# XuyangGuo/CtrlHair

Hardware: AMD Instinct MI355X
Metric: 512x512 edited images/sec (SEAN generator forward), whole job (higher is better)
Workload: dtype f32 (every product and sum an IEEE f32 operation on the f32 matrix cores, v_mfma_f32_16x16x4_f32 / 32x32x2_f32; 3x3 convs as Winograd: ResBlock convs and the <= 64-pixel SPADE / style convs F(4x4,3x3), SPADE / style convs above F(2x2,3x3) -- f32 operands and accumulation over TRANSFORMED operands, n; 1 GPU; SEAN generator forward only, batch 16/GPU, 512x512, ngf=64 (BASELINE.json configs[1] per GPU); global_batch=16, parallelism=batch-sharded x1, labels=blocky, spade_interior_reduction=True

## Files before the change

ctrlhair_amd/csrc/ch_api.cpp:

```cpp
#include "../../include/ctrlhair_hip.h"

#include <hip/hip_runtime.h>

#include <algorithm>
#include <cmath>
#include <cstdint>
#include <cstring>
#include <new>
#include <string>

#include "aux_models.h"
#include "sean_model.h"
#include "kernels.h"
#include "png_inflate_core.h"

struct ch_handle {
    int device = 0;
    std::string err;
    chk::TensorStore tensors[4];
    chk::SeanModel sean;
    bool sean_ready = false;
    chk::ShapeModel shape;
    chk::ColorModel color;
    chk::BiSeNetModel bisenet;
// ... 643 lines not shown
int ch_sean_set_tap(ch_handle* h, const char* name, float* dev_ptr) {
    if (!h || !name) return CH_ERR_ARG;
    if (dev_ptr) h->sean.taps[name] = dev_ptr;
    else h->sean.taps.erase(name);
    return CH_OK;
}

int ch_sean_scale_report(ch_handle* h, float* host_out, int n) {
    if (!h || !host_out || n < 0) return CH_ERR_ARG;
    if (!h->sean_ready || !h->sean.amax_slots) return fail(h, CH_ERR_STATE, "ch_sean_scale_report: SEAN weights not finalized");
    DeviceGuard guard(h->device);
    unsigned raw[64];
    if (hipDeviceSynchronize() != hipSuccess ||
        hipMemcpy(raw, h->sean.amax_slots, sizeof raw, hipMemcpyDeviceToHost) != hipSuccess)
        return fail(h, CH_ERR_HIP, "ch_sean_scale_report: device read failed");
    for (int i = 0; i < n; ++i) {
        float v = 0.f;
        if (i < 64) std::memcpy(&v, &raw[i], 4);
        host_out[i] = v;
    }
    return CH_OK;
}

int ch_sean_debug_read(ch_handle* h, void* host_out, size_t bytes) {
    if (!h || !host_out) return CH_ERR_ARG;
    if (!h->sean_ready || !h->sean.splitk_ws) return fail(h, CH_ERR_STATE, "ch_sean_debug_read: SEAN weights not finalized");
    DeviceGuard guard(h->device);
    if ((long long)bytes > h->sean.splitk_cap * 4) return fail(h, CH_ERR_ARG, "ch_sean_debug_read: too many bytes");
    if (hipDeviceSynchronize() != hipSuccess || hipMemcpy(host_out, h->sean.splitk_ws, bytes, hipMemcpyDeviceToHost) != hipSuccess)
        return fail(h, CH_ERR_HIP, "ch_sean_debug_read: device read failed");
    return CH_OK;
}

}

namespace {
enum OptFreeze { NEVER, BY_SEAN, BY_SHAPE, BY_BISENET };
enum OptMap { BOOL, CLAMP, RAW };
struct OptRow {
    const char* key;
    OptFreeze frozen_by;
    OptMap map;
    int lo, hi;
    void (*set)(ch_handle*, int);
    int (*guard)(ch_handle*, int);
};
constexpr int MAXI = 0x7fffffff;
#define OPT_FIELD(field) [](ch_handle* h, int v) { h->field = v; }, nullptr
#define SEAN_FIELD(field) OPT_FIELD(sean.opt.field)

int guard_sparse(ch_handle* h, int value) {
    if (h->sean_ready && value != 0 && !h->sean.gtab)
        return fail(h, CH_ERR_STATE, "ch_set_option(sean.sparse = 1): the handle was finalised with sean.sparse = 0 (no buffers); set it before ch_finalize");
    return CH_OK;
}
int guard_dbg(ch_handle* h, int value) {
#ifndef CH_ABLATE
    if (value & CH_ABLATE_DBG_MASK)
        return fail(h, CH_ERR_ARG, "ch_set_option(sean.dbg): timing-ablation / superseded-kernel bits need a library built with -DCH_ABLATE "
                                   "(make -C ctrlhair_amd/csrc ABLATE=1)");
#endif
    return CH_OK;
}

const OptRow OPTION_TABLE[] = {
    {"sean.f16x3", BY_SEAN, RAW, 0, 0, [](ch_handle* h, int v) { h->sean.opt.use_sh16 = v != 0; h->sean.opt.terms = v == 2 ? 1 : (v == 3 ? 2 : 3); }, nullptr},
    {"shape.f16x3", BY_SHAPE, BOOL, 0, 0, OPT_FIELD(shape.use_sh16)},
    {"shape.overlap", BY_SHAPE, BOOL, 0, 0, OPT_FIELD(shape.overlap)},
    {"shape.enc_lut", BY_SHAPE, BOOL, 0, 0, OPT_FIELD(shape.enc_l0_lut)},
    {"bisenet.f16x3", BY_BISENET, BOOL, 0, 0, OPT_FIELD(bisenet.use_sh16)},
    {"aux.wino", NEVER, BOOL, 0, 0, [](ch_handle* h, int v) { h->shape.wino = h->bisenet.wino = v; }, nullptr},
    {"sean.ahead", BY_SEAN, RAW, 0, 0, [](ch_handle* h, int v) { h->sean.opt.ahead_pixels = (long long)v * 512 * 512; }, nullptr},
    {"sean.wino", BY_SEAN, CLAMP, 0, 2, SEAN_FIELD(wino)},
    {"sean.lut_grouped", BY_SEAN, BOOL, 0, 0, SEAN_FIELD(lut_grouped)},
    {"sean.prologue", BY_SEAN, BOOL, 0, 0, SEAN_FIELD(prologue)},
    {"sean.overlap", BY_SEAN, CLAMP, 0, MAXI, SEAN_FIELD(overlap)},
    {"sean.wino4_force", NEVER, BOOL, 0, 0, SEAN_FIELD(wino4_force)},
    {"sean.patch", BY_SEAN, BOOL, 0, 0, SEAN_FIELD(patch)},
    {"sean.convt_gemm", BY_SEAN, BOOL, 0, 0, SEAN_FIELD(convt_gemm)},
    {"sean.edge", BY_SEAN, BOOL, 0, 0, SEAN_FIELD(edge)},
    {"sean.frame", BY_SEAN, BOOL, 0, 0, SEAN_FIELD(frame)},
    {"sean.int_groups", NEVER, CLAMP, 0, MAXI, SEAN_FIELD(int_groups)},
    {"sean.int_onepass", NEVER, BOOL, 0, 0, SEAN_FIELD(int_onepass)},
    {"sean.batch_invariant", NEVER, BOOL, 0, 0, SEAN_FIELD(batch_inv)},
    {"sean.wino4v", BY_SEAN, BOOL, 0, 0, SEAN_FIELD(wino4v)},
    {"sean.wino4_split", BY_SEAN, CLAMP, -1, 1, SEAN_FIELD(wino4_split)},
    {"sean.wino4_ace", BY_SEAN, CLAMP, 0, MAXI, SEAN_FIELD(wino4_ace_max_r)},
    {"sean.hidden_wq", NEVER, BOOL, 0, 0, SEAN_FIELD(hidden_wq)},
    {"sean.wino_gather", BY_SEAN, BOOL, 0, 0, SEAN_FIELD(wino_gather)},
    {"sean.wino_th", BY_SEAN, RAW, 0, 0, SEAN_FIELD(wino_th)},
    {"sean.sparse", NEVER, BOOL, 0, 0, [](ch_handle* h, int v) { h->sean.opt.sparse = v; }, guard_sparse},
    {"sean.sh16_compact", BY_SEAN, CLAMP, 0, 2, SEAN_FIELD(sh16_compact)},
    {"sean.sparse_th", BY_SEAN, RAW, 0, 0, SEAN_FIELD(sparse_th)},
    {"sean.sparse_min", BY_SEAN, RAW, 0, 0, SEAN_FIELD(sparse_min_r)},
    {"sean.dbg_sel", NEVER, RAW, 0, 0, SEAN_FIELD(dbg_sel)},
    {"sean.dbg", NEVER, RAW, 0, 0, [](ch_handle* h, int v) { h->sean.opt.dbg = v; }, guard_dbg},
};
#undef SEAN_FIELD
#undef OPT_FIELD
}

extern "C" {

int ch_set_option(ch_handle* h, const char* key, int value) {
    if (!h || !key) return CH_ERR_ARG;
    for (const OptRow& r : OPTION_TABLE) {
        if (std::strcmp(key, r.key) != 0) continue;
        const bool frozen = r.frozen_by == BY_SEAN ? h->sean_ready : r.frozen_by == BY_SHAPE ? h->shape.ready : r.frozen_by == BY_BISENET && h->bisenet.ready;
        if (frozen) return fail(h, CH_ERR_STATE, std::string("ch_set_option(") + key + ") must precede ch_finalize");
        if (int rc = r.guard ? r.guard(h, value) : CH_OK) return rc;
        r.set(h, r.map == BOOL ? value != 0 : (r.map == CLAMP ? std::max(r.lo, std::min(r.hi, value)) : value));
        return CH_OK;
    }
    return fail(h, CH_ERR_ARG, std::string("unknown option '") + key + "'");
}

int ch_mfma_peak(ch_handle* h, int kind, int ms_target, double* tflops) {
    if (!h || !tflops || kind < 0 || kind > 1 || ms_target < 1 || ms_target > 2000) return fail(h, CH_ERR_ARG, "ch_mfma_peak: bad argument");
    DeviceGuard guard(h->device);
    hipError_t e = chk::mfma_peak(kind, ms_target, tflops, nullptr);
    return e == hipSuccess ? CH_OK : fail(h, CH_ERR_HIP, std::string("ch_mfma_peak: ") + hipGetErrorString(e));
}

int ch_profile_enable(ch_handle* h, int on) {
    if (!h) return CH_ERR_ARG;
    h->sean.prof_on = on != 0;
    return CH_OK;
}

int ch_profile_read(ch_handle* h, int kind, int* launches, double* total_ms, double* flops, double* bytes) {
    return ch_profile_read_ex(h, kind, launches, total_ms, flops, nullptr, bytes);
}

int ch_profile_read_ex(ch_handle* h, int kind, int* launches, double* total_ms, double* flops, double* flops_executed,
                       double* bytes) {
    if (!h) return CH_ERR_ARG;
    DeviceGuard guard(h->device);
    int n = 0;
    double ms = 0, fl = 0, fx = 0, by = 0;
    for (auto& r : h->sean.prof) {
        if (hipEventSynchronize(r.e1) != hipSuccess) return fail(h, CH_ERR_HIP, "hipEventSynchronize failed");
        if (kind < 0 || r.kind == kind) {
            float t = 0.f;
            if (hipEventElapsedTime(&t, r.e0, r.e1) != hipSuccess) return fail(h, CH_ERR_HIP, "hipEventElapsedTime failed");
            ms += t;
            fl += r.flops;
            if (r.sp_stat) {
                int st[4] = {0, 0, 0, 0};
                if (hipMemcpy(st, r.sp_stat, sizeof st, hipMemcpyDeviceToHost) != hipSuccess)
                    return fail(h, CH_ERR_HIP, "ch_profile_read: work-list statistics read failed");
                fx += (double)st[3] * r.sp_flops_unit;
                by += r.sp_bytes_fixed + r.sp_bytes_px * (r.kind == 3 ? r.sp_npix - (double)st[1] : (double)st[1]);
            } else {
                fx += r.flops_exec >= 0.0 ? r.flops_exec : r.flops;
                by += r.bytes;
            }
            ++n;
        }
    }
    if (flops_executed) *flops_executed = fx;
    if (kind < 0) {
        for (auto& r : h->sean.prof) {
            h->sean.ev_pool.push_back(r.e0);
            h->sean.ev_pool.push_back(r.e1);
        }
        h->sean.prof.clear();
// ... 11 lines not shown
```

ctrlhair_amd/csrc/conv_inst_wino.hip:

```cpp
#include "conv_pw.h"
#include <algorithm>
#include "conv_wino.h"

namespace chk {

static int wino_num_cus() {
    static int cus[64] = {};
    int dev = 0;
    if (hipGetDevice(&dev) != hipSuccess || dev < 0 || dev >= 64) return 256;
    if (!cus[dev]) {
        int v = 0;
        if (hipDeviceGetAttribute(&v, hipDeviceAttributeMultiprocessorCount, dev) != hipSuccess || v <= 0) v = 256;
        cus[dev] = v;
    }
    return cus[dev];
}

template <class K>
static hipError_t wino_attr(K kern, int bytes, bool (&done)[64]) {
    int dev = 0;
    if (hipGetDevice(&dev) != hipSuccess || dev < 0 || dev >= 64) return hipErrorInvalidDevice;
    if (!done[dev]) {
        hipError_t e = hipFuncSetAttribute(reinterpret_cast<const void*>(kern), hipFuncAttributeMaxDynamicSharedMemorySize, bytes);
        if (e != hipSuccess) return e;
// ... 10 lines not shown
        for (int k = 1; k < ks; ++k) {
            const float4 t = reinterpret_cast<const float4*>(partial + k * slab)[i];
            a.x += t.x; a.y += t.y; a.z += t.z; a.w += t.w;
        }
        const long long e = 4 * i;
        const int x = (int)(e % W), y = (int)((e / W) % H);
        const long long bc = e / ((long long)W * H);
        const float bv = bias ? bias[bc % C] : 0.f;
        a.x += bv; a.y += bv; a.z += bv; a.w += bv;
        if (res) {
            if (res_up) {
                const float* rp = res + bc * (long long)(H >> 1) * (W >> 1) + (long long)(y >> 1) * (W >> 1) + (x >> 1);
                a.x += rp[0]; a.y += rp[0]; a.z += rp[1]; a.w += rp[1];
            } else {
                const float4 r = reinterpret_cast<const float4*>(res)[i];
                a.x += r.x; a.y += r.y; a.z += r.z; a.w += r.w;
            }
        }
        if (act != ACT_NONE) { a.x = apply_act(a.x, act); a.y = apply_act(a.y, act); a.z = apply_act(a.z, act); a.w = apply_act(a.w, act); }
        reinterpret_cast<float4*>(out)[i] = a;
    }
}

hipError_t conv_wino_plain(WinoParams p, hipStream_t s) {
    if ((!wino_supported(p.H, p.W, p.Cin) && !(wino_supported_pair16(p.B, p.H, p.W, p.Cin) && !p.reflect && !p.res_up)) || !p.zero) return hipErrorInvalidValue;
    if (p.d2s && (p.Cout % 4 || p.res || p.reflect || p.in_up || !wino_supported(p.H, p.W, p.Cin))) return hipErrorInvalidValue;
    if (p.in_up && (p.reflect || !wino_supported(p.H, p.W, p.Cin))) return hipErrorInvalidValue;
    wino_fill_launch(p);
    p.ksplit = 1;
    if (p.partial && !p.d2s && p.W % 4 == 0) {
        const int cus = wino_num_cus();
        int ks = 1;
        while (ks < 8 && 2 * ks * p.ntasks <= cus && p.nks % (2 * ks) == 0 && p.nks / (2 * ks) >= 16 &&
               (long long)2 * ks * p.B * p.Cout * p.H * p.W <= p.partial_cap)
            ks *= 2;
        if (ks > 1) {
            p.ksplit = ks;
            p.ntasks *= ks;
        }
    }
    if (p.nks / p.ksplit < wino::NST) p.claim = nullptr;
    const int grid = p.ntasks < wino_num_cus() ? p.ntasks : wino_num_cus();
    static bool d0[64] = {}, d1[64] = {}, d2[64] = {};
    if (p.d2s) {
        hipError_t e = wino_attr(wino_plain_kernel<1>, wino::LDS_BYTES, d1);
        if (e != hipSuccess) return e;
        hipLaunchKernelGGL(wino_plain_kernel<1>, dim3(grid), dim3(512), wino::LDS_BYTES, s, p);
        return hipGetLastError();
    }
    if (p.in_up) {
        hipError_t e = wino_attr(wino_plain_kernel<2>, wino::LDS_BYTES, d2);
        if (e != hipSuccess) return e;
        hipLaunchKernelGGL(wino_plain_kernel<2>, dim3(grid), dim3(512), wino::LDS_BYTES, s, p);
    } else {
        hipError_t e = wino_attr(wino_plain_kernel<0>, wino::LDS_BYTES, d0);
        if (e != hipSuccess) return e;
        hipLaunchKernelGGL(wino_plain_kernel<0>, dim3(grid), dim3(512), wino::LDS_BYTES, s, p);
    }
    if (p.ksplit > 1) {
        const long long n4 = (long long)p.B * p.Cout * p.H * p.W / 4;
        const int blocks = (int)std::min<long long>((n4 + 255) / 256, 4096);
        hipLaunchKernelGGL(wino_splitk_reduce_kernel, dim3(blocks), dim3(256), 0, s, p.partial, p.out, p.bias, p.res, p.res_up, p.act, p.ksplit, p.B, p.Cout, p.H,
                           p.W);
    }
    return hipGetLastError();
}


template <int RT>
static hipError_t launch_pw(PwParams p, hipStream_t s) {
    using Cfg = PwCfg<RT>;
    static bool d0[64] = {};
    hipError_t e = wino_attr(pw_conv_kernel<RT>, Cfg::LDS_BYTES, d0);
    if (e != hipSuccess) return e;
    const int nrt = (p.Cout + 31) / 32;
    p.nrg = (nrt + RT - 1) / RT;
    p.npt = p.HW / Cfg::PXB;
    p.ntasks = p.B * p.npt * p.nrg;
    p.nst = p.Cin / 16;
    const int grid = p.ntasks < wino_num_cus() ? p.ntasks : wino_num_cus();
    hipLaunchKernelGGL(pw_conv_kernel<RT>, dim3(grid), dim3(512), Cfg::LDS_BYTES, s, p);
    return hipGetLastError();
}
hipError_t conv_pw(PwParams p, hipStream_t s) {
    if (!pw_supported(p.Cin, p.Cout, p.HW)) return hipErrorInvalidValue;
    p.groups = nullptr;
    p.ngroups = 0;
    return (p.Cout + 31) / 32 >= 4 ? launch_pw<4>(p, s) : launch_pw<2>(p, s);
}
hipError_t conv_pw_grouped(PwParams p, int ntasks, hipStream_t s) {
    using Cfg = PwCfg<4>;
    if (p.Cin % 16 || p.Cout < 1 || !p.groups || p.ngroups < 1 || ntasks < 1) return hipErrorInvalidValue;
    static bool d0[64] = {};
    hipError_t e = wino_attr(pw_conv_kernel<4>, Cfg::LDS_BYTES, d0);
    if (e != hipSuccess) return e;
    p.in = p.wpk = nullptr;
    p.out = nullptr;
    p.B = 1;
    p.HW = 0;
    p.nrg = ((p.Cout + 31) / 32 + 3) / 4;
    p.npt = 0;
    p.ntasks = ntasks;
    p.nst = p.Cin / 16;
    const int grid = ntasks < wino_num_cus() ? ntasks : wino_num_cus();
    hipLaunchKernelGGL(pw_conv_kernel<4>, dim3(grid), dim3(512), Cfg::LDS_BYTES, s, p);
    return hipGetLastError();
}

template <int TH>
static hipError_t launch_wino_ace(const WinoAceParams& p, hipStream_t s) {
    static bool d0[64] = {};
    hipError_t e = wino_attr(wino_ace_kernel<TH>, WaCfg<TH>::LDS_BYTES, d0);
    if (e != hipSuccess) return e;
    hipLaunchKernelGGL(wino_ace_kernel<TH>, dim3(wino_num_cus()), dim3(512), WaCfg<TH>::LDS_BYTES, s, p);
    return hipGetLastError();
}
hipError_t conv_wino_ace(WinoAceParams p, hipStream_t s) {
    if (p.gq) {
        if (!p.gq_n || p.gq_cap <= 0 || p.B > 32 || !p.work || !p.total || (p.C & 3) || (p.W & 1) || (p.H & 1)) return hipErrorInvalidValue;
        p.nrt = (p.C + 15) / 16;
        if (p.nrt > 2 * 65535) return hipErrorInvalidValue;
        p.K = 128 + (p.wsty ? 20 : 0);
        static bool d0[64] = {};
        hipError_t e = wino_attr(wino_ace_gather_kernel<0>, winog::LDS_BYTES, d0);
        if (e != hipSuccess) return e;
        hipLaunchKernelGGL(wino_ace_gather_kernel<0>, dim3(wino_num_cus()), dim3(512), winog::LDS_BYTES, s, p);
        return hipGetLastError();
    }
    if ((p.TH != 16 && p.TH != 32) || p.H % p.TH || p.W % wino::TW || !p.zero || !p.qlist || !p.qcnt || !p.work || !p.total || (p.C & 3))
        return hipErrorInvalidValue;
    p.nrt = (p.C + 15) / 16;
    p.ntx = p.W / wino::TW;
    p.nty = p.H / p.TH;
    p.K = 128 + (p.wsty ? 20 : 0);
    return p.TH == 32 ? launch_wino_ace<32>(p, s) : launch_wino_ace<16>(p, s);
}

__device__ __forceinline__ void wino_gather_scan_block(const int* __restrict__ qcnt, int* __restrict__ qoff, int* __restrict__ gq_n, int tps, int b) {
    __shared__ int wsum[16];
    __shared__ int carry;
    const int tid = threadIdx.x, lane = tid & 63, wave = tid >> 6;
    if (tid == 0) carry = 0;
    __syncthreads();
    for (int t0 = 0; t0 < tps; t0 += 1024) {
        const int t = t0 + tid;
        const int c = t < tps ? qcnt[b * tps + t] : 0;
        int v = c;
#pragma unroll
        for (int off = 1; off < 64; off <<= 1) {
            const int u = __shfl_up(v, off, 64);
            if (lane >= off) v += u;
        }
        if (lane == 63) wsum[wave] = v;
        __syncthreads();
        int base = carry;
        for (int w = 0; w < wave; ++w) base += wsum[w];
        if (t < tps) qoff[b * tps + t] = base + v - c;
        __syncthreads();
        if (tid == 1023) carry = base + v;
        __syncthreads();
    }
    if (tid == 0) gq_n[b] = carry;
}
__global__ __launch_bounds__(1024) void wino_gather_scan_kernel(const int* __restrict__ qcnt, int* __restrict__ qoff, int* __restrict__ gq_n, int tps) {
    wino_gather_scan_block(qcnt, qoff, gq_n, tps, (int)blockIdx.x);
}
__device__ __forceinline__ void wino_gather_fill_block(const uint8_t* __restrict__ qlist, const int* __restrict__ qcnt, const int* __restrict__ qoff,
                                                       unsigned* __restrict__ gq, int gq_cap, int ntx, int nty, int tile) {
    const int i = threadIdx.x;
    if (i >= qcnt[tile]) return;
    const int b = tile / (ntx * nty), tr = tile % (ntx * nty);
    const int q = qlist[(long long)tile * 128 + i];
    const unsigned y = (unsigned)((tr / ntx) * 16 + 2 * (q >> 4)), x = (unsigned)((tr % ntx) * 32 + 2 * (q & 15));
    gq[(long long)b * gq_cap + qoff[tile] + i] = y << 16 | x;
}
__global__ __launch_bounds__(128) void wino_gather_fill_kernel(const uint8_t* __restrict__ qlist, const int* __restrict__ qcnt, const int* __restrict__ qoff,
                                                               unsigned* __restrict__ gq, int gq_cap, int ntx, int nty) {
    wino_gather_fill_block(qlist, qcnt, qoff, gq, gq_cap, ntx, nty, (int)blockIdx.x);
}
hipError_t wino_gather_lists(const uint8_t* qlist, const int* qcnt, int* qoff, unsigned* gq, int* gq_n, int gq_cap, int B, int H, int W, hipStream_t s) {
    if (H % 16 || W % 32 || B > 32 || H > 65535 || W > 65535) return hipErrorInvalidValue;
    const int ntx = W / 32, nty = H / 16;
    hipLaunchKernelGGL(wino_gather_scan_kernel, dim3(B), dim3(1024), 0, s, qcnt, qoff, gq_n, ntx * nty);
    hipLaunchKernelGGL(wino_gather_fill_kernel, dim3(B * ntx * nty), dim3(128), 0, s, qlist, qcnt, qoff, gq, gq_cap, ntx, nty);
    return hipGetLastError();
}
__device__ __forceinline__ void wino_gather_worklist_block(const int* __restrict__ gq_n, const int* __restrict__ pcnt, int B, int tps, int nrt,
                                                           unsigned* __restrict__ work, int* __restrict__ total) {
// ... 265 lines not shown
```

ctrlhair_amd/csrc/conv_inst_wino4.hip:

```cpp
#include "conv_wino4v.h"
#include "conv_wino4_split.h"

namespace chk {

hipError_t conv_wino4_plain(Wino4Params p, hipStream_t s) {
    if (!wino4_supported(p.H, p.W, p.Cin) || !p.in || !p.wpk || !p.out || (p.reflect && (p.res_up || p.H < 2 || p.W < 2))) return hipErrorInvalidValue;
    wino4_fill_launch(p);
    static bool done[64] = {};
    static int cus[64] = {};
    int dev = 0;
    if (hipGetDevice(&dev) != hipSuccess || dev < 0 || dev >= 64) return hipErrorInvalidDevice;
    if (!done[dev]) {
        hipError_t e = hipFuncSetAttribute(reinterpret_cast<const void*>(wino4_plain_kernel<0>), hipFuncAttributeMaxDynamicSharedMemorySize, wino4::LDS_BYTES);
        if (e != hipSuccess) return e;
        e = hipFuncSetAttribute(reinterpret_cast<const void*>(wino4_plain_kernel<1>), hipFuncAttributeMaxDynamicSharedMemorySize, wino4::LDS_BYTES);
        if (e != hipSuccess) return e;
        e = hipFuncSetAttribute(reinterpret_cast<const void*>(wino4_plain_split_kernel<0>), hipFuncAttributeMaxDynamicSharedMemorySize, wino4::LDS_BYTES);
        if (e != hipSuccess) return e;
        e = hipFuncSetAttribute(reinterpret_cast<const void*>(wino4_plain_split_kernel<1>), hipFuncAttributeMaxDynamicSharedMemorySize, wino4::LDS_BYTES);
        if (e != hipSuccess) return e;
        int v = 0;
        if (hipDeviceGetAttribute(&v, hipDeviceAttributeMultiprocessorCount, dev) != hipSuccess || v <= 0) v = 256;
        cus[dev] = v;
        done[dev] = true;
    }
    const int grid = p.ntasks < cus[dev] ? p.ntasks : cus[dev];
    if (p.wpk_split && (p.split > 0 || (p.split < 0 && wino4_split_pays(p)))) {
        if (p.nks & 1) return hipErrorInvalidValue;
        if (p.reflect) hipLaunchKernelGGL(wino4_plain_split_kernel<1>, dim3(grid), dim3(512), wino4::LDS_BYTES, s, p);
        else hipLaunchKernelGGL(wino4_plain_split_kernel<0>, dim3(grid), dim3(512), wino4::LDS_BYTES, s, p);
        return hipGetLastError();
    }
    if (p.reflect) hipLaunchKernelGGL(wino4_plain_kernel<1>, dim3(grid), dim3(512), wino4::LDS_BYTES, s, p);
    else hipLaunchKernelGGL(wino4_plain_kernel<0>, dim3(grid), dim3(512), wino4::LDS_BYTES, s, p);
    return hipGetLastError();
}

hipError_t conv_wino4_ace(Wino4AceParams p, hipStream_t s) {
    if (!wino4_ace_supported(p.H, p.W, p.C) || !p.actv || !p.wpk || !p.out || !p.x || !p.noise) return hipErrorInvalidValue;
    p.nrt = (p.C + 15) / 16;
    p.ntx = p.W / wino4::TS;
    p.nty = p.H / wino4::TS;
    p.ntiles = p.B * p.ntx * p.nty;
    p.ntasks = p.ntiles * p.nrt;
    p.nks = p.wsty ? 38 : 32;
    p.rb = p.nrt >= 4 ? 4 : p.nrt;
    p.tbk = 32 / p.rb;
    static bool done[64] = {};
    static int cus[64] = {};
    int dev = 0;
    if (hipGetDevice(&dev) != hipSuccess || dev < 0 || dev >= 64) return hipErrorInvalidDevice;
    if (!done[dev]) {
        hipError_t e = hipFuncSetAttribute(reinterpret_cast<const void*>(wino4_ace_kernel<0>), hipFuncAttributeMaxDynamicSharedMemorySize, wino4::LDS_BYTES);
        if (e != hipSuccess) return e;
        int v = 0;
        if (hipDeviceGetAttribute(&v, hipDeviceAttributeMultiprocessorCount, dev) != hipSuccess || v <= 0) v = 256;
        cus[dev] = v;
        done[dev] = true;
    }
    const int grid = p.ntasks < cus[dev] ? p.ntasks : cus[dev];
    hipLaunchKernelGGL(wino4_ace_kernel<0>, dim3(grid), dim3(512), wino4::LDS_BYTES, s, p);
    return hipGetLastError();
}

__global__ __launch_bounds__(256) void wino4_style_pack_kernel(const float* __restrict__ lut, float* __restrict__ wsty, int B, int C, int nrt) {
    const long long n = (long long)B * nrt * 6 * 1152;
    const long long i = blockIdx.x * 256LL + threadIdx.x;
    if (i >= n) return;
    const int lane = (int)(i & 63), idx = (int)((i >> 6) % 18), s = (int)((i / 1152) % 6);
    const int rt = (int)((i / (1152 * 6)) % nrt), b = (int)(i / (1152LL * 6 * nrt));
    const int j = 4 * s + (lane >> 4);
    float4 o = make_float4(0.f, 0.f, 0.f, 0.f);
    const int m = (4 * idx) / 36;
    int ch, beta;
    wino4_ace_row(rt * 32 + m * 16 + (lane & 15), ch, beta);
    if (ch < C && j < 19 && s < 5) {
        const float* P = lut + ((long long)(b * 19 + j) * 9) * 2 * C + beta * C + ch;
        float g[3][3];
#pragma unroll
        for (int t = 0; t < 9; ++t) g[t / 3][t % 3] = P[(long long)t * 2 * C];
        const float Gm[6][3] = {{0.25f, 0.f, 0.f}, {-1.f / 6, -1.f / 6, -1.f / 6}, {-1.f / 6, 1.f / 6, -1.f / 6},
                                {1.f / 24, 1.f / 12, 1.f / 6}, {1.f / 24, -1.f / 12, 1.f / 6}, {0.f, 0.f, 1.f}};
        float u[4];
#pragma unroll
        for (int e = 0; e < 4; ++e) {
            const int xi = 4 * idx + e - 36 * m, ii = xi / 6, jj = xi % 6;
            float r[3];
#pragma unroll
            for (int q = 0; q < 3; ++q) r[q] = Gm[ii][0] * g[0][q] + Gm[ii][1] * g[1][q] + Gm[ii][2] * g[2][q];
            u[e] = r[0] * Gm[jj][0] + r[1] * Gm[jj][1] + r[2] * Gm[jj][2];
        }
        o = make_float4(u[0], u[1], u[2], u[3]);
    }
    reinterpret_cast<float4*>(wsty)[i] = o;
}
hipError_t wino4_style_pack(const float* lut, float* wsty, int B, int C, hipStream_t s) {
    const int nrt = (C + 15) / 16;
    const long long n = (long long)B * nrt * 6 * 1152;
    hipLaunchKernelGGL(wino4_style_pack_kernel, dim3((unsigned)((n + 255) / 256)), dim3(256), 0, s, lut, wsty, B, C, nrt);
    return hipGetLastError();
}


static hipError_t wino4v_device(int& cus) {
    static bool done[64] = {};
    static int ncu[64] = {};
    int dev = 0;
    if (hipGetDevice(&dev) != hipSuccess || dev < 0 || dev >= 64) return hipErrorInvalidDevice;
    if (!done[dev]) {
        hipError_t e = hipFuncSetAttribute(reinterpret_cast<const void*>(wino4v_kernel<0>), hipFuncAttributeMaxDynamicSharedMemorySize, wino4v::LDS_BYTES);
        if (e != hipSuccess) return e;
        e = hipFuncSetAttribute(reinterpret_cast<const void*>(wino4v_kernel<1>), hipFuncAttributeMaxDynamicSharedMemorySize, wino4v::LDS_BYTES);
        if (e != hipSuccess) return e;
        int v = 0;
        if (hipDeviceGetAttribute(&v, hipDeviceAttributeMultiprocessorCount, dev) != hipSuccess || v <= 0) v = 256;
        ncu[dev] = v;
        done[dev] = true;
    }
    cus = ncu[dev];
    return hipSuccess;
}
hipError_t wino4v_pack(const Wino4vPackParams& p, hipStream_t s) {
    if (!p.in || !p.v || p.H % 32 || p.W % 32 || p.H < 32 || p.W < 32 || p.nks <= 0 || p.pitch % 4 || p.xoff % 4 || (p.reflect && p.padded)) return hipErrorInvalidValue;
    const long long blocks = (long long)p.B * (p.H / 32) * (p.W / 32) * p.nks;
    if (blocks <= 0 || blocks > 0x7fffffffLL) return hipErrorInvalidValue;
    hipLaunchKernelGGL(wino4v_pack_kernel<0>, dim3((unsigned)blocks), dim3(256), 0, s, p);
    return hipGetLastError();
}
hipError_t conv_wino4v_plain(Wino4Params p, hipStream_t s) {
    if (!wino4_supported(p.H, p.W, p.Cin) || !p.v || !p.wpk || !p.out) return hipErrorInvalidValue;
    wino4_fill_launch(p);
    if (p.nks & 1) return hipErrorInvalidValue;
#ifndef W4V_RB
#define W4V_RB 8
#endif
    p.rb = p.nrt >= W4V_RB ? W4V_RB : p.nrt;
    p.tbk = 32 / p.rb;
    int cus = 0;
    hipError_t e = wino4v_device(cus);
    if (e != hipSuccess) return e;
    const int grid = p.ntasks < cus ? p.ntasks : cus;
    hipLaunchKernelGGL(wino4v_kernel<0>, dim3(grid), dim3(512), wino4v::LDS_BYTES, s, p);
    return hipGetLastError();
}
hipError_t conv_wino4v_ace(Wino4AceParams p, hipStream_t s) {
    if (!wino4_ace_supported(p.H, p.W, p.C) || !p.v || !p.wpk || !p.out || !p.x || !p.noise) return hipErrorInvalidValue;
    p.nrt = (p.C + 15) / 16;
    p.ntx = p.W / wino4::TS;
    p.nty = p.H / wino4::TS;
    p.ntiles = p.B * p.ntx * p.nty;
    p.ntasks = p.ntiles * p.nrt;
    p.nks = p.wsty ? 38 : 32;
    p.rb = p.nrt >= 4 ? 4 : p.nrt;
    p.tbk = 32 / p.rb;
    int cus = 0;
    hipError_t e = wino4v_device(cus);
    if (e != hipSuccess) return e;
    const int grid = p.ntasks < cus ? p.ntasks : cus;
    hipLaunchKernelGGL(wino4v_kernel<1>, dim3(grid), dim3(512), wino4v::LDS_BYTES, s, p);
    return hipGetLastError();
}

}
```

ctrlhair_amd/csrc/conv_pw.h:

```cpp
#pragma once
#include "conv_wino.h"

namespace chk {

struct PwGroup {
    const float* in;
    const float* wpk;
    float* out;
    int HW, start;
};
struct PwParams {
    const float* in;
    const float* wpk;
    float* out;
    int B, Cin, Cout, HW;
    const PwGroup* groups;
    int ngroups;
    long long in_bs;
    int nrg, npt, ntasks, nst;
};

template <class F>
std::vector<float> pack_pw_A(int rows, int Cin, F get) {
    const int nrt = (rows + 31) / 32, nst = Cin / 16;
    std::vector<float> dst((size_t)nrt * nst * 512, 0.f);
    for (int rt = 0; rt < nrt; ++rt)
        for (int st = 0; st < nst; ++st)
            for (int lane = 0; lane < 64; ++lane)
                for (int s = 0; s < 8; ++s) {
                    const int row = rt * 32 + (lane & 31), ci = 16 * st + 2 * s + (lane >> 5);
                    if (row < rows) dst[((size_t)rt * nst + st) * 512 + lane * 8 + s] = get(row, ci);
                }
    return dst;
}

template <int RT>
struct PwCfg {
    static constexpr int PG = 8 / RT, PXB = 64 * PG;
    static constexpr int PDW = 16 * PXB, ADW = RT * 512;
    static constexpr int SDW = PDW + ADW, NST = 6;
    static constexpr int NPD = PDW / (4 * 512);
    static constexpr int NLD = NPD + 1;
    static constexpr int LDS_BYTES = NST * SDW * 4 + 512 * 16;
};

template <int RT>
__global__ __launch_bounds__(512, 1) void pw_conv_kernel(const PwParams p) {
    using Cfg = PwCfg<RT>;
    constexpr int PG = Cfg::PG, PXB = Cfg::PXB, PDW = Cfg::PDW, SDW = Cfg::SDW, NST = Cfg::NST, NPD = Cfg::NPD, NLD = Cfg::NLD;
    extern __shared__ __attribute__((aligned(16))) float smem[];
    const int tid = threadIdx.x, lane = tid & 63;
    const int wave = __builtin_amdgcn_readfirstlane(tid >> 6);
    const int G = gridDim.x;
    const int lb = xcd_remap(blockIdx.x, G);
    if (lb >= p.ntasks) return;
    const int mytasks = (p.ntasks - lb + G - 1) / G;
    const int nst = p.nst;
    constexpr unsigned SB = SDW * 4, RING = NST * SB;
    auto group_of = [&](int L) {
        int g = 0;
        while (g + 1 < p.ngroups && L >= p.groups[g + 1].start * p.nrg) ++g;
        return g;
    };
    const unsigned lds0 = (unsigned)(size_t)(wino_lds_void*)smem;

    unsigned vp[NPD];
    const bool a_wave = wave < RT * 2;
    int it = lb, is = 0;
    wino_u32x4 d_in, d_a;
    unsigned so_in = 0, so_a = 0;
    int HW = p.HW;
    auto issue_task = [&]() {
        int rg, pt, ib;
        const float *tin, *twpk;
        if (p.groups) {
            const int g = group_of(it), local = it - p.groups[g].start * p.nrg;
            rg = local % p.nrg;
            pt = local / p.nrg;
            ib = 0;
            HW = p.groups[g].HW;
            tin = p.groups[g].in;
            twpk = p.groups[g].wpk;
        } else {
            rg = it % p.nrg;
            pt = (it / p.nrg) % p.npt;
            ib = it / (p.nrg * p.npt);
            tin = p.in;
            twpk = p.wpk;
        }
#pragma unroll
        for (int i = 0; i < NPD; ++i) {
            const int u = i * 512 + tid, ch = u / (PXB / 4), q = u - ch * (PXB / 4);
            vp[i] = (unsigned)(ch * HW + pt * PXB + 4 * q) * 4u;
        }
        d_in = wino_rsrc(tin + (long long)ib * (p.in_bs ? p.in_bs : (long long)p.Cin * HW), (unsigned)p.Cin * HW * 4u);
        const int nrt = (p.Cout + 31) / 32, have = nrt - rg * RT < RT ? nrt - rg * RT : RT;
        d_a = wino_rsrc(twpk + (long long)rg * RT * nst * 512, (unsigned)have * nst * 2048u);
        so_in = 0;
        so_a = 0;
    };
    issue_task();
    const unsigned va_rt = a_wave ? (unsigned)((tid >> 7) * nst * 2048 + (tid & 127) * 16) : 0x80000000u;
    unsigned islot = lds0;
    auto issue = [&]() {
        const unsigned wb = islot + (unsigned)wave * 1024u;
#pragma unroll
        for (int i = 0; i < NPD; ++i) wino_dma16(vp[i], d_in, so_in, wb + (unsigned)i * 8192u);
        const unsigned wa = a_wave ? islot + PDW * 4u + (unsigned)wave * 1024u : lds0 + RING + (unsigned)wave * 1024u;
        wino_dma16(va_rt, d_a, so_a, wa);
        islot = islot + SB == lds0 + RING ? lds0 : islot + SB;
        so_in += 64u * (unsigned)HW;
        so_a += 2048u;
        if (++is == nst) {
            if (it + G < p.ntasks) {
                it += G;
                is = 0;
                issue_task();
            } else {
                is = nst - 1;
                so_in -= 64u * (unsigned)HW;
                so_a -= 2048u;
            }
        }
    };

    f32x16 acc[2];
#pragma unroll
    for (int n = 0; n < 2; ++n)
#pragma unroll
        for (int r = 0; r < 16; ++r) acc[n][r] = 0.f;
    const int rtl = wave / PG, pg = wave % PG;
    const int boff = (lane >> 5) * PXB + pg * 64 + (lane & 31);
    const int aoff = PDW + rtl * 512 + lane * 8;

#pragma unroll
    for (int j = 0; j < NST - 1; ++j) issue();
    asm volatile("s_waitcnt vmcnt(%0)" ::"n"(NLD * (NST - 3)) : "memory");
    __syncthreads();
    unsigned rslot = lds0;
    bool after_epi = false;
    auto frag = [&](unsigned slot) { return reinterpret_cast<const float*>(smem) + (slot - lds0) / 4; };
    float4 a_lo = *reinterpret_cast<const float4*>(frag(lds0) + aoff), a_hi = *reinterpret_cast<const float4*>(frag(lds0) + aoff + 4);
    float b0 = frag(lds0)[boff], b1 = frag(lds0)[boff + 32];
    for (int k = 0, ct = lb; k < mytasks; ++k, ct += G) {
        for (int cs = 0; cs < nst; ++cs) {
            if (after_epi) asm volatile("s_waitcnt vmcnt(0)" ::: "memory");
            else asm volatile("s_waitcnt vmcnt(%0)" ::"n"(NLD * (NST - 3)) : "memory");
            __syncthreads();
            after_epi = false;
            issue();
            const unsigned nslot = rslot + SB == lds0 + RING ? lds0 : rslot + SB;
            const float* sp = frag(rslot);
            const float* spn = frag(nslot);
            const float av[8] = {a_lo.x, a_lo.y, a_lo.z, a_lo.w, a_hi.x, a_hi.y, a_hi.z, a_hi.w};
#pragma unroll
            for (int s = 0; s < 8; ++s) {
                const float c0 = b0, c1 = b1;
                if (s < 7) {
                    b0 = sp[boff + (2 * s + 2) * PXB];
                    b1 = sp[boff + (2 * s + 2) * PXB + 32];
                } else {
                    b0 = spn[boff];
                    b1 = spn[boff + 32];
                    a_lo = *reinterpret_cast<const float4*>(spn + aoff);
                    a_hi = *reinterpret_cast<const float4*>(spn + aoff + 4);
                }
                acc[0] = __builtin_amdgcn_mfma_f32_32x32x2f32(av[s], c0, acc[0], 0, 0, 0);
                acc[1] = __builtin_amdgcn_mfma_f32_32x32x2f32(av[s], c1, acc[1], 0, 0, 0);
            }
            rslot = nslot;
        }
        {
            int rg, pt, b, eHW;
            float* tout;
            if (p.groups) {
                const int g = group_of(ct), local = ct - p.groups[g].start * p.nrg;
                rg = local % p.nrg;
                pt = local / p.nrg;
                b = 0;
                eHW = p.groups[g].HW;
                tout = p.groups[g].out;
            } else {
                rg = ct % p.nrg;
                pt = (ct / p.nrg) % p.npt;
                b = ct / (p.nrg * p.npt);
                eHW = p.HW;
                tout = p.out;
            }
            const int row0 = (rg * RT + rtl) * 32 + 4 * (lane >> 5);
            float* ob = tout + (long long)b * p.Cout * eHW + pt * PXB + pg * 64 + (lane & 31);
#pragma unroll
            for (int n = 0; n < 2; ++n)
#pragma unroll
                for (int r = 0; r < 16; ++r) {
                    const int row = row0 + (r & 3) + 8 * (r >> 2);
                    if (row < p.Cout) ob[(long long)row * eHW + n * 32] = acc[n][r];
                    acc[n][r] = 0.f;
                }
            after_epi = true;
        }
    }
    asm volatile("s_waitcnt vmcnt(0)" ::: "memory");
}

inline bool pw_supported(int Cin, int Cout, int HW) { return Cin % 16 == 0 && HW % 256 == 0 && Cout >= 32; }
hipError_t conv_pw(PwParams p, hipStream_t s);
inline int pw_group_tasks(int Cout, int HW) { return ((((Cout + 31) / 32) + 3) / 4) * (HW / 128); }
hipError_t conv_pw_grouped(PwParams p, int ntasks, hipStream_t s);

}
```

ctrlhair_amd/csrc/conv_wino4.h:

```cpp
#pragma once
#include "conv_wino.h"

namespace chk {

namespace wino4 {
constexpr int TS = 32;
constexpr int PROWS = 34, PUN = 10;
constexpr int PPL = PROWS * PUN;
constexpr int PUNITS = 4 * PPL;
constexpr int PSLOTS = 1408;
constexpr int AUNITS = 1152;
constexpr int SUNITS = PSLOTS + AUNITS;
constexpr int NST = 4;
constexpr int LDS_BYTES = NST * SUNITS * 16;
constexpr int ADW = AUNITS * 4;
}

struct Wino4Params {
    const float* in;
    const float* wpk;
    float* out;
    int B, Cin, Cout, H, W;
    const float* bias;
    const float* res;
// ... 535 lines not shown
    issue_kstep();
    issue_kstep();
    asm volatile("s_waitcnt vmcnt(0)" ::: "memory");
    __syncthreads();
    unsigned rslot = lds0;
    auto kstep = [&](float (&vc)[36], float (&vx)[36]) {
        wait_ring();
        __syncthreads();
        const unsigned nslot = rslot + SB == lds0 + RING ? lds0 : rslot + SB;
        const f32x4* ap = a_ptr(rslot);
        const float* spn = stage(nslot);
        wino4_lds_f2* hbn = wino4_halo_base(spn + boff + 5);
        f32x4 F[2];
        F[0] = ap[0];
        float d[6];
        auto group = [&](auto gt) {
            constexpr int g = decltype(gt)::value;
            if constexpr (g + 1 < 9) F[(g + 1) & 1] = ap[(g + 1) * 64];
            if constexpr (g < 6) load_row(spn, hbn, g, d);
            __builtin_amdgcn_sched_barrier(0);
            const f32x4 c = F[g & 1];
            __builtin_amdgcn_s_setprio(1);
            acc[4 * g] = __builtin_amdgcn_mfma_f32_16x16x4f32(c.x, vc[4 * g], acc[4 * g], 0, 0, 0);
            acc[4 * g + 1] = __builtin_amdgcn_mfma_f32_16x16x4f32(c.y, vc[4 * g + 1], acc[4 * g + 1], 0, 0, 0);
            acc[4 * g + 2] = __builtin_amdgcn_mfma_f32_16x16x4f32(c.z, vc[4 * g + 2], acc[4 * g + 2], 0, 0, 0);
            acc[4 * g + 3] = __builtin_amdgcn_mfma_f32_16x16x4f32(c.w, vc[4 * g + 3], acc[4 * g + 3], 0, 0, 0);
            __builtin_amdgcn_s_setprio(0);
            if constexpr (g < 6)
                wino4_in1d(d[0], d[1], d[2], d[3], d[4], d[5], vx[6 * g], vx[6 * g + 1], vx[6 * g + 2], vx[6 * g + 3], vx[6 * g + 4], vx[6 * g + 5]);
            if constexpr (g >= 6) {
#pragma unroll
                for (int j = 2 * (g - 6); j < 2 * (g - 6) + 2; ++j)
                    wino4_in1d(vx[j], vx[6 + j], vx[12 + j], vx[18 + j], vx[24 + j], vx[30 + j], vx[j], vx[6 + j], vx[12 + j], vx[18 + j], vx[24 + j],
                               vx[30 + j]);
            }
            __builtin_amdgcn_sched_barrier(0);
            if constexpr (g >= 2 && g < 6) issue_piece(WInt<g - 2>{});
            __builtin_amdgcn_sched_barrier(0);
        };
        group(WInt<0>{}); group(WInt<1>{}); group(WInt<2>{}); group(WInt<3>{}); group(WInt<4>{}); group(WInt<5>{});
        group(WInt<6>{}); group(WInt<7>{}); group(WInt<8>{});
        issue_tail();
        rslot = nslot;
    };

    for (int k = 0, ct = lb; k < mytasks; ++k, ct += G) {
        {
            float v[36], w[36];
            first_v(rslot, v);
            for (int cs = 0; cs < nk; cs += 2) {
                kstep(v, w);
                kstep(w, v);
            }
        }
        int crt, tile;
        task_of(ct, crt, tile);
        wino4_ace_epilogue(p, acc, crt, tile, mh, kk, tyl, tx);
#pragma unroll
        for (int x2 = 0; x2 < 36; ++x2) acc[x2] = (f32x4){0.f, 0.f, 0.f, 0.f};
        asm volatile("s_waitcnt vmcnt(0)" ::: "memory");
    }
}

inline bool wino4_supported(int H, int W, int Cin) { return H % wino4::TS == 0 && W % wino4::TS == 0 && Cin % 8 == 0 && Cin >= 16; }
inline bool wino4_pays(long long ntasks4, int cus) {
    if (cus <= 0) cus = 256;
    const long long r4 = (ntasks4 + cus - 1) / cus, r2 = (2 * ntasks4 + cus - 1) / cus;
    return r4 * 36 * 68 < r2 * 32 * 58;
}
inline void wino4_fill_launch(Wino4Params& p) {
    p.nrt = (p.Cout + 31) / 32;
    p.ntx = p.W / wino4::TS;
    p.nty = p.H / wino4::TS;
    p.ntiles = p.B * p.ntx * p.nty;
    p.ntasks = p.ntiles * p.nrt;
    p.nks = p.Cin / 4;
    p.rb = p.nrt >= 4 ? 4 : p.nrt;
    p.tbk = 32 / p.rb;
}
inline bool wino4_split_pays(const Wino4Params& p) { return p.Cin >= 128; }
hipError_t conv_wino4_plain(Wino4Params p, hipStream_t s);
inline bool wino4_ace_supported(int H, int W, int C) { return H % wino4::TS == 0 && W % wino4::TS == 0 && C % 2 == 0; }
hipError_t conv_wino4_ace(Wino4AceParams p, hipStream_t s);
hipError_t wino4_style_pack(const float* lut, float* wsty, int B, int C, hipStream_t s);

}
```

ctrlhair_amd/csrc/kernels.h:

```cpp
#pragma once
#include <hip/hip_runtime.h>
#include <stdint.h>

#include <map>
#include <utility>
#include <vector>

namespace chk {
hipError_t label_downsample(const uint8_t* in, uint8_t* out, int B, int S, int r, hipStream_t s);
hipError_t onehot_conv3x3(const uint8_t* lab, const float* table, const float* bias, float* out, int B, int H, int W,
                          int K, int relu, hipStream_t s, int c4 = 0, const uint8_t* need = nullptr, int kout = 0);
hipError_t label_onehot_planes(const uint8_t* lab, float* out, int B, int H, int W, int kout, int k0, hipStream_t s);
bool spade_hidden_wq_supported(int H, int W);
hipError_t ace_finish_f32(const float* gb, int rowsP, const float* x, int x_up, const float* bias_g, const float* bias_b, const float* bn_a,
                          const float* bn_d, const float* nv, const float* noise, long long noise_bstride, const uint8_t* lab, const float* lut,
                          float* out, int B, int C, int H, int W, int act, hipStream_t s);
hipError_t spade_hidden_wq(const uint8_t* lab, const uint8_t* u5, const float* table, const float* bias, float* out, int B, int H, int W,
                           int kout, int onehot, hipStream_t s, int pitch = 0, int xoff = 0, const int* skip_if_patch = nullptr);
struct HiddenGroup {
    static constexpr int MAX = 24;
    struct Entry {
        const uint8_t* lab;
        const uint8_t* u5;
        const float* table;
        const float* bias;
        float* out;
        int H, W, kout, onehot, pitch, xoff;
        int tcs, start, nblk;
    };
    Entry e[MAX];
    int n, B;
};
hipError_t spade_hidden_wq_grouped(HiddenGroup& g, hipStream_t s);
hipError_t spade_hidden_patch(const uint8_t* lab, const unsigned* gq, const int* gq_n, int gq_cap, const int* chunk_base, const int* mode,
                              const float* table, const float* bias, float* patch, int B, int H, int W, int kout, hipStream_t s);
hipError_t spade_hidden_level(const uint8_t* lab, const uint8_t* u5, const unsigned* gq, const int* gq_n, int gq_cap, const int* chunk_base, const int* mode,
                              const float* table, const float* bias, float* out, float* patch, int B, int H, int W, int kout, int onehot, int pitch,
                              int xoff, hipStream_t s);
hipError_t wino_chunk_base(const int* gq_n, int B, int cap_chunks, int* chunk_base, int* mode, hipStream_t s);
hipError_t onehot_conv3x3_sh16(const uint8_t* lab, const float* table, const float* bias, void* out, int B, int H, int W,
                               int K, int relu, float scale, hipStream_t s, int bf16 = 0, const uint8_t* need = nullptr,
                               const int* tile_cnt = nullptr,
                               int need_impl = 0);
hipError_t sh16_decode(const void* in, float* out, int B, int C, long long HW, float scale, const unsigned* amax,
                       hipStream_t s, int bf16 = 0, int single = 0);
hipError_t fc_mu(const float* codes, const float* Wt, const float* bias, float* mu_img, int B, int Npad, hipStream_t s,
                 float* mu_rows = nullptr, int sh16 = 0, int bs = 19, float scale = 1.f, unsigned* amax = nullptr,
                 int pass = 0, int bf16 = 0);
hipError_t fc_mu_batched(const float* codes, const float* const* Wts, const float* const* biases, float* mu_base,
                         long long mu_stride, int n_aces, int B, int Npad, int bs, float scale, unsigned* amax_slots, int pass,
                         int bf16, hipStream_t s, int sh16 = 1);
hipError_t conv_img_tanh(const float* x, const float* w, const float* bias, float* out, int B, int Cin, int H, int W,
                         hipStream_t s, int c4 = 0, const float* w4 = nullptr);
hipError_t c4_decode(const float* in, float* out, int B, int C, long long HW, hipStream_t s);
hipError_t gen_noise(float* out, long long n, uint64_t seed, hipStream_t s);
hipError_t mfma_peak(int kind, int ms_target, double* tflops, hipStream_t s);
float instnorm_sh16_scale(int HW);
hipError_t instnorm_act(float* x, int planes, int HW, float eps, int act, hipStream_t s, void* sh16 = nullptr, int C = 0,
                        float* scratch = nullptr);
hipError_t convt_shift4(const float* x, float* xs, int B, int C, int H, int W, hipStream_t s);
hipError_t instnorm_act_d2s(const float* t, const float* bias, float* out, int B, int C, int H, int W, float eps, int act, hipStream_t s);
hipError_t instnorm_c4_to_sh16(const float* x_c4, int B, int C, int HW, float eps, int act, void* sh16, hipStream_t s,
                               float* scratch = nullptr);
hipError_t layernorm_act(float* x, const float* gamma, const float* beta, float* part, int B, int C, int HW, float eps,
                         int act, hipStream_t s);
hipError_t layernorm_act_conv(const float* x, int in_c4, void* out, int out_sh16, float out_scale, const float* gamma,
                              const float* beta, float* part, int B, int C, int HW, float eps, int act, hipStream_t s);
hipError_t region_mean(const float* codes, const uint8_t* lab, float* out, int B, int F, int h, int w, int S,
                       hipStream_t s, int c4 = 0);
hipError_t maxpool3x3s2(const float* in, float* out, long long planes, int H, int W, hipStream_t s);
hipError_t global_avg_pool(const float* in, float* out, int planes, int HW, hipStream_t s);
hipError_t chan_affine(const float* in, const float* sc, float sc_add, const float* sh, const float* other, float* out,
                       long long planes, int HW, hipStream_t s);
hipError_t stem7x7(const float* in, const float* w, const float* bias, float* out, int B, int H, int W, hipStream_t s);
hipError_t conv3x3_c3_reflect(const float* in, const float* w, const float* bias, float* out, int B, int Cout, int H, int W,
                              hipStream_t s);
hipError_t bilinear_argmax(const float* lg, uint8_t* out, float* logits_out, const uint8_t* remap, int B, int h, int w,
                           int H, int W, hipStream_t s, int c4 = 0);
hipError_t maxpool3x3s2_c4(const float* in_nchw, float* out_c4, unsigned* amax, int B, int C, int H, int W, hipStream_t s);
hipError_t global_avg_pool_c4(const float* in, float* out, int B, int C, int HW, hipStream_t s);
hipError_t chan_affine_c4(const float* in, const float* sc, float sc_add, const float* sh, const float* other, float* out,
                          unsigned* amax, int B, int C, int HW, hipStream_t s);
hipError_t shape_softmax(const float* hair, const float* face, uint8_t* lab, float* probs, int B, int HW, hipStream_t s,
                         int c4 = 0);
hipError_t c4_rows_to_nchw(const float* in, float* out, int B, int C, int Cpad, int HW, hipStream_t s);
hipError_t shape_enc_l0(const uint8_t* lab, const float* tab, const float* pc_hair, const float* pc_face, float* out_hair, float* out_face,
                        int B, int S, hipStream_t s);
hipError_t shape_inputs(const uint8_t* lab, const float* pos, float* hair_in, float* face_in, int B, int HW,
                        hipStream_t s);
hipError_t shape_inputs_sh16(const uint8_t* lab, const float* pos, void* hair_in, void* face_in, int B, int HW, float scale,
                             hipStream_t s);
hipError_t linear(const float* x, const float* W, const float* bias, const float* scale, const float* shift, float* out,
                  int B, int K, int O, int ldx, int ldo, int act, hipStream_t s);
hipError_t lut_gemv_mfma(const float* x, const float* W, float* out, int N, int rows, hipStream_t s);
hipError_t subspace_add(float* h, const float* z, int zld, const float* U, const float* L, const float* mu, int B, int D,
                        int Z, hipStream_t s);
size_t poisson_workspace_bytes(int H, int W);
hipError_t poisson_blend_batch(const uint8_t* src_hwc, const uint8_t* tgt_hwc, const uint8_t* mask, uint8_t* out_hwc, int B, int H, int W,
                               int with_gamma, int max_iters, double rel_tol, void* ws, int* iters_out, hipStream_t s);
hipError_t blend_mask_batch(const uint8_t* target_parsing, const uint8_t* face_parsing, uint8_t* out, int B, int H, int W, hipStream_t s);

constexpr int HAIR_ERODE_MAX_R = 15;
constexpr int HAIR_COLOR_NSTAT = 22;
struct HairErodeRows {
    int r;
    int hw[2 * HAIR_ERODE_MAX_R + 1];
};
hipError_t resize_linear_u8(const uint8_t* src, uint8_t* dst, int B, int Hs, int Ws, int C, int Hd, int Wd, hipStream_t s);
hipError_t hair_erode(const uint8_t* labels, int B, int Hl, int Wl, int label, const HairErodeRows& rows, uint8_t* mask, int H, int W,
                      hipStream_t s);
hipError_t hair_color_stats(const uint8_t* img, const uint8_t* mask, int B, int H, int W, int64_t* sums, hipStream_t s);

constexpr int SWEEP_NSTAT = 16;
hipError_t sheet_compose(const void* src, int kind, int n, int Hs, int Ws, const int* cells, const uint8_t* lut, uint8_t* canvas, int rows,
                         int cols, int H, int W, int margin, hipStream_t s);
hipError_t sweep_stats(const void* img, int kind, const uint8_t* labels, const int* ref, int N, int H, int W, int h, int w, int64_t* stats,
                       hipStream_t s);

constexpr int WARP_MAX_V = 2048;
constexpr int WARP_MAX_F = 4096;
constexpr int WARP_DESC_PAIRS = 16;
struct WarpDesc {
    int n, pair0;
    int d[WARP_DESC_PAIRS][6];
};
size_t mask_warp_workspace_bytes(int B);
hipError_t mask_warp_batch(const uint8_t* hair_labels, const uint8_t* face_labels, const float* V, const int* F, const int* bidx,
                           const float* bc, const int* desc_host, const float* U_in, uint8_t* labels_out, float* uv_out, float* U_out,
                           void* ws, int B, int outer_iters, int max_cg, float rel_tol, hipStream_t s);
hipError_t mask_warp_batch_dev(const uint8_t* hair_labels, const uint8_t* face_labels, const float* V, const int* F, const int* bidx,
                               const float* bc, const int* desc_dev, const float* U_in, uint8_t* labels_out, float* uv_out, float* U_out,
                               void* ws, int B, int outer_iters, int max_cg, float rel_tol, hipStream_t s);

constexpr int DELAUNAY_DESC_SETS = 64;
// ... 72 lines not shown
```

ctrlhair_amd/csrc/sean_kernels.hip:

```cpp
#include "kernels.h"
#include "sh16.h"

namespace chk {

constexpr int AF_CG = 8;
__global__ __launch_bounds__(256) void ace_finish_f32_kernel(const float* __restrict__ gb, int rowsP, const float* __restrict__ x, int x_up,
                                                             const float* __restrict__ bias_g, const float* __restrict__ bias_b,
                                                             const float* __restrict__ bn_a, const float* __restrict__ bn_d,
                                                             const float* __restrict__ nv, const float* __restrict__ noise, long long noise_bstride,
                                                             const uint8_t* __restrict__ lab, const float* __restrict__ lut, float* __restrict__ out,
                                                             int B, int C, int H, int W, int act) {
    const int HW = H * W, ppb = (HW + 255) / 256;
    const int b = blockIdx.x / ppb, pix = (blockIdx.x - b * ppb) * 256 + threadIdx.x;
    if (pix >= HW) return;
    const int y = pix / W, xx = pix - y * W;
    const int c0 = blockIdx.y * AF_CG;
    const int xW = W >> x_up, xHW = xW * (H >> x_up);
    const float nz = noise[(long long)b * noise_bstride + (long long)xx * H + y];
    const float* xp = x + ((long long)b * C + c0) * xHW + (y >> x_up) * xW + (xx >> x_up);
    const float* gp = gb + (long long)b * rowsP * HW + pix;
    float* op = out + ((long long)b * C + c0) * HW + pix;
    unsigned lo[9];
    unsigned lmask = 0;
    const float* Lb = lut ? lut + (long long)b * 19 * 9 * 2 * C : nullptr;
// ... 695 lines not shown
                        const float4 r0 = rr[0], r1 = rr[1];
                        a0.x += r0.x; a0.y += r0.y; a0.z += r0.z; a0.w += r0.w;
                        a1.x += r1.x; a1.y += r1.y; a1.z += r1.z; a1.w += r1.w;
                    }
                }
                const float v8[8] = {a0.x, a0.y, a0.z, a0.w, a1.x, a1.y, a1.z, a1.w};
                h8 vh, vl;
#pragma unroll
                for (int e2 = 0; e2 < 8; ++e2) {
                    float v = v8[e2];
                    if (relu) v = v > 0.f ? v : 0.f;
                    if (k0 + gq * 8 + e2 >= K) v = 0.f;
                    _Float16 h, l;
                    sh16_split_any(v, scale, bf16, h, l);
                    vh[e2] = h;
                    vl[e2] = l;
                }
                const long long unit = (((long long)b * G + g) * 2) * HW + pix;
                typedef unsigned u32x4 __attribute__((ext_vector_type(4)));
                __builtin_nontemporal_store(__builtin_bit_cast(u32x4, vh), reinterpret_cast<u32x4*>(out + unit));
                __builtin_nontemporal_store(__builtin_bit_cast(u32x4, vl), reinterpret_cast<u32x4*>(out + unit + HW));
            }
        }
        __syncthreads();
        if (threadIdx.x == 0) pcount = 0;
        __syncthreads();
    }
}

hipError_t onehot_conv3x3_sh16(const uint8_t* lab, const float* table, const float* bias, void* out, int B, int H, int W,
                               int K, int relu, float scale, hipStream_t s, int bf16, const uint8_t* need, const int* tile_cnt,
                               int need_impl) {
    if (need && !tile_cnt && (need_impl == 0 ? W >= 512 : need_impl == 2)) {
        const int ntile = B * ((W + 31) / 32) * ((H + 31) / 32), ky = (K + OH_KC - 1) / OH_KC;
        int gx = 1280 / ky;
        if (gx > ntile) gx = ntile;
        hipLaunchKernelGGL(onehot_conv3x3_sh16_need_kernel, dim3((unsigned)gx, (unsigned)ky), dim3(256), 0, s, lab, table, bias,
                           static_cast<uint4*>(out), B, H, W, K, relu, scale, bf16, need);
        return hipGetLastError();
    }
    const long long npix = (long long)B * H * W;
    dim3 grid((unsigned)((npix + 255) / 256), (unsigned)((K + OH_KC - 1) / OH_KC));
    hipLaunchKernelGGL(onehot_conv3x3_sh16_kernel, grid, dim3(256), 0, s, lab, table, bias, static_cast<uint4*>(out), B, H,
                       W, K, relu, scale, bf16, need, tile_cnt);
    return hipGetLastError();
}

__global__ void sh16_decode_kernel(const _Float16* __restrict__ in, float* __restrict__ out, int B, int C, long long HW,
                                   float inv_scale, const unsigned* __restrict__ amax, int bf16, int single) {
    if (amax) inv_scale /= sh16_dyn_extra(*amax);
    const long long n = (long long)B * C * HW;
    const int G = (C + 7) / 8;
    for (long long i = blockIdx.x * (long long)blockDim.x + threadIdx.x; i < n; i += (long long)gridDim.x * blockDim.x) {
        const long long p = i % HW;
        const int c = (int)((i / HW) % C), b = (int)(i / (HW * C));
        const long long unit = (((long long)b * G + c / 8) * 2) * HW + p;
        if (bf16) out[i] = (float)__builtin_bit_cast(__bf16, in[unit * 8 + (c & 7)]) * inv_scale;
        else if (single) out[i] = (float)in[unit * 8 + (c & 7)] * inv_scale;
        else out[i] = ((float)in[unit * 8 + (c & 7)] + (float)in[(unit + HW) * 8 + (c & 7)]) * inv_scale;
    }
}
hipError_t sh16_decode(const void* in, float* out, int B, int C, long long HW, float scale, const unsigned* amax,
                       hipStream_t s, int bf16, int single) {
    hipLaunchKernelGGL(sh16_decode_kernel, dim3(4096), dim3(256), 0, s, static_cast<const _Float16*>(in), out, B, C, HW,
                       1.f / scale, amax, bf16, single);
    return hipGetLastError();
}

__global__ void c4_decode_kernel(const float* __restrict__ in, float* __restrict__ out, int B, int C, long long HW) {
    const long long n = (long long)B * C * HW;
    for (long long i = blockIdx.x * (long long)blockDim.x + threadIdx.x; i < n; i += (long long)gridDim.x * blockDim.x) {
        const long long p = i % HW;
        const int c = (int)((i / HW) % C), b = (int)(i / (HW * C));
        out[i] = in[(((long long)b * (C >> 2) + (c >> 2)) * HW + p) * 4 + (c & 3)];
    }
}
hipError_t c4_decode(const float* in, float* out, int B, int C, long long HW, hipStream_t s) {
    hipLaunchKernelGGL(c4_decode_kernel, dim3(4096), dim3(256), 0, s, in, out, B, C, HW);
    return hipGetLastError();
}

constexpr int FCMU_BT = 8;

__device__ __forceinline__ void fc_mu_body(const float* __restrict__ codes, const float* __restrict__ Wt,
                                           const float* __restrict__ bias, float* __restrict__ mu_img, int B, int Npad,
                                           float* __restrict__ mu_rows, int sh16, int bs, float scale,
                                           unsigned* __restrict__ amax, int pass, int bf16, int bx, int j) {
    sh16_mode_on();
    if (sh16 == 1 && amax && pass == 1) {
        const float e = sh16_dyn_extra(*amax);
        if (e == 1.f) return;
        scale *= e;
    }
    float vmax = 0.f;
    const int wave = threadIdx.x >> 6, lane = threadIdx.x & 63;
    const int o0 = (bx * 4 + wave) * 4;
    const float* Wj = Wt + (long long)j * 512 * 512;
    float4 w[4][2];
#pragma unroll
    for (int i = 0; i < 4; ++i) {
        const float4* wr = reinterpret_cast<const float4*>(Wj + (long long)(o0 + i) * 512 + lane * 8);
        w[i][0] = wr[0];
        w[i][1] = wr[1];
    }
    for (int bb = 0; bb < B; bb += FCMU_BT) {
        float part[4][FCMU_BT];
#pragma unroll
        for (int t = 0; t < FCMU_BT; ++t) {
            float4 c0 = make_float4(0, 0, 0, 0), c1 = c0;
            if (bb + t < B) {
                const float4* cr =
                    reinterpret_cast<const float4*>(codes + ((long long)(bb + t) * 19 + j) * 512 + lane * 8);
                c0 = cr[0];
                c1 = cr[1];
            }
#pragma unroll
            for (int i = 0; i < 4; ++i)
                part[i][t] = w[i][0].x * c0.x + w[i][0].y * c0.y + w[i][0].z * c0.z + w[i][0].w * c0.w +
                             w[i][1].x * c1.x + w[i][1].y * c1.y + w[i][1].z * c1.z + w[i][1].w * c1.w;
        }
#pragma unroll
        for (int i = 0; i < 4; ++i)
#pragma unroll
            for (int t = 0; t < FCMU_BT; ++t) {
                float v = part[i][t];
#pragma unroll
                for (int off = 32; off > 0; off >>= 1) v += __shfl_xor(v, off, 64);
                part[i][t] = v;
            }
        if (lane == 0) {
#pragma unroll
            for (int i = 0; i < 4; ++i)
#pragma unroll
                for (int t = 0; t < FCMU_BT; ++t)
                    if (bb + t < B) {
                        const float v = part[i][t] + bias[j * 512 + o0 + i];
                        const float r = v > 0.f ? v : 0.f;
                        const int o = o0 + i, n = (bb + t) * bs + j;
                        if (bs > 19 && j == 0) {
                            const int nz = (bb + t) * bs + 19;
                            if (mu_rows) mu_rows[(long long)nz * 512 + o] = 0.f;
                            else if (sh16 == 1) {
                                _Float16* mh = reinterpret_cast<_Float16*>(mu_img);
                                mh[(((long long)(o >> 3) * 2 + 0) * Npad + nz) * 8 + (o & 7)] = (_Float16)0.f;
                                mh[(((long long)(o >> 3) * 2 + 1) * Npad + nz) * 8 + (o & 7)] = (_Float16)0.f;
                            }
                        }
                        if (mu_rows) mu_rows[(long long)n * 512 + o] = r;
                        else if (sh16 == 2)
                            mu_img[((long long)(n >> 5) * 32 + (o >> 4)) * 512 + ((n & 31) + 32 * (o & 1)) * 8 + ((o & 15) >> 1)] = r;
                        else if (sh16) {
                            _Float16* mh = reinterpret_cast<_Float16*>(mu_img);
                            _Float16 h, l;
                            sh16_split_any(r, scale, bf16, h, l);
                            vmax = fmaxf(vmax, r * scale);
                            mh[(((long long)(o >> 3) * 2 + 0) * Npad + n) * 8 + (o & 7)] = h;
                            mh[(((long long)(o >> 3) * 2 + 1) * Npad + n) * 8 + (o & 7)] = l;
                        } else mu_img[(long long)o * Npad + n] = r;
                    }
        }
    }
    if (sh16 == 1 && amax && pass == 0 && lane == 0) sh16_slot_max(amax, vmax);
}
__global__ __launch_bounds__(256) void fc_mu_kernel(const float* __restrict__ codes, const float* __restrict__ Wt,
                                                    const float* __restrict__ bias, float* __restrict__ mu_img, int B,
                                                    int Npad, float* __restrict__ mu_rows, int sh16, int bs, float scale,
                                                    unsigned* __restrict__ amax, int pass, int bf16) {
    fc_mu_body(codes, Wt, bias, mu_img, B, Npad, mu_rows, sh16, bs, scale, amax, pass, bf16, blockIdx.x, blockIdx.y);
}
__global__ __launch_bounds__(256) void fc_mu_batched_kernel(const float* __restrict__ codes, const float* const* __restrict__ Wts,
                                                            const float* const* __restrict__ biases, float* __restrict__ mu_base,
                                                            long long mu_stride, int B, int Npad, int bs, float scale,
                                                            unsigned* __restrict__ amax_slots, int pass, int bf16, int sh16) {
    const int a = blockIdx.z;
    const float* Wt = Wts[a];
    if (!Wt) return;
    fc_mu_body(codes, Wt, biases[a], mu_base + a * mu_stride, B, Npad, nullptr, sh16, bs, scale, sh16 == 1 ? amax_slots + 2 * a + 1 : nullptr, pass,
               bf16, blockIdx.x, blockIdx.y);
}
hipError_t fc_mu_batched(const float* codes, const float* const* Wts, const float* const* biases, float* mu_base,
                         long long mu_stride, int n_aces, int B, int Npad, int bs, float scale, unsigned* amax_slots, int pass,
                         int bf16, hipStream_t s, int sh16) {
    hipLaunchKernelGGL(fc_mu_batched_kernel, dim3(512 / 16, 19, n_aces), dim3(256), 0, s, codes, Wts, biases, mu_base, mu_stride, B,
                       Npad, bs, scale, amax_slots, pass, bf16, sh16);
    return hipGetLastError();
}

hipError_t fc_mu(const float* codes, const float* Wt, const float* bias, float* mu_img, int B, int Npad,
                 hipStream_t s, float* mu_rows, int sh16, int bs, float scale, unsigned* amax, int pass, int bf16) {
    hipLaunchKernelGGL(fc_mu_kernel, dim3(512 / 16, 19), dim3(256), 0, s, codes, Wt, bias, mu_img, B, Npad, mu_rows, sh16, bs,
                       scale, amax, pass, bf16);
    return hipGetLastError();
}

constexpr int CI_TW = 32, CI_TH = 8, CI_CK = 8;

__global__ __launch_bounds__(256) void conv_img_kernel(const float* __restrict__ x, const float* __restrict__ w,
                                                       const float* __restrict__ bias, float* __restrict__ out, int B,
                                                       int Cin, int H, int W, int c4) {
    __shared__ float patch[CI_CK][CI_TH + 2][CI_TW + 2];
    const int tx = threadIdx.x % CI_TW, ty = threadIdx.x / CI_TW;
    const int x0 = blockIdx.x * CI_TW, y0 = blockIdx.y * CI_TH, b = blockIdx.z;
    const long long HW = (long long)H * W;
    float a0 = 0.f, a1 = 0.f, a2 = 0.f;
    for (int c0 = 0; c0 < Cin; c0 += CI_CK) {
        __syncthreads();
        for (int e = threadIdx.x; e < CI_CK * (CI_TH + 2) * (CI_TW + 2); e += 256) {
            const int c = e / ((CI_TH + 2) * (CI_TW + 2)), rem = e % ((CI_TH + 2) * (CI_TW + 2));
            const int py = rem / (CI_TW + 2), px = rem % (CI_TW + 2);
            const int yy = y0 + py - 1, xx = x0 + px - 1;
            float v = 0.f;
            if (c0 + c < Cin && (unsigned)yy < (unsigned)H && (unsigned)xx < (unsigned)W) {
                const int ch = c0 + c;
                v = c4 ? x[(((long long)b * (Cin >> 2) + (ch >> 2)) * HW + (long long)yy * W + xx) * 4 + (ch & 3)]
                       : x[((long long)b * Cin + ch) * HW + (long long)yy * W + xx];
                v = v > 0.f ? v : 0.2f * v;
            }
            patch[c][py][px] = v;
        }
        __syncthreads();
        const float* w0 = w + (long long)c0 * 9;
#pragma unroll
        for (int c = 0; c < CI_CK; ++c) {
            if (c0 + c >= Cin) break;
#pragma unroll
            for (int t = 0; t < 9; ++t) {
                const float v = patch[c][ty + t / 3][tx + t % 3];
                a0 += w0[c * 9 + t] * v;
                a1 += w0[(long long)Cin * 9 + c * 9 + t] * v;
                a2 += w0[(long long)Cin * 18 + c * 9 + t] * v;
            }
        }
    }
    const int xx = x0 + tx, yy = y0 + ty;
    if (xx < W && yy < H) {
        float* o = out + (long long)b * 3 * HW + (long long)yy * W + xx;
        o[0] = tanhf(a0 + bias[0]);
        o[HW] = tanhf(a1 + bias[1]);
        o[2 * HW] = tanhf(a2 + bias[2]);
    }
}

template <bool NCHW>
__global__ __launch_bounds__(256) void conv_img_c4_kernel(const float4* __restrict__ x, const float4* __restrict__ w4,
                                                          const float* __restrict__ bias, float* __restrict__ out, int B,
                                                          int Cin, int H, int W) {
    constexpr int PW = CI_TW + 2, PH = CI_TH + 2, NP = PW * PH;
    __shared__ float4 patch[2][NP];
    const int G = Cin >> 2;
    const int tx = threadIdx.x % CI_TW, ty = threadIdx.x / CI_TW;
    const int x0 = blockIdx.x * CI_TW, y0 = blockIdx.y * CI_TH, b = blockIdx.z;
    const long long HW = (long long)H * W;
    int off[2];
#pragma unroll
    for (int i = 0; i < 2; ++i) {
        const int e = threadIdx.x + i * 256;
        const int py = e / PW, px = e % PW, yy = y0 + py - 1, xx = x0 + px - 1;
        off[i] = (e < NP && (unsigned)yy < (unsigned)H && (unsigned)xx < (unsigned)W) ? yy * W + xx : -1;
    }
    const float4* xb = x + (long long)b * G * HW;
    const float* xp = reinterpret_cast<const float*>(x) + (long long)b * Cin * HW;
    float4 r[2];
    auto fetch = [&](int g) {
#pragma unroll
        for (int i = 0; i < 2; ++i) {
            float4 v;
            if constexpr (NCHW) {
                const float* q = xp + (long long)(4 * g) * HW + (off[i] >= 0 ? off[i] : 0);
                v = make_float4(q[0], q[HW], q[2 * HW], q[3 * HW]);
            } else {
                v = xb[(long long)g * HW + (off[i] >= 0 ? off[i] : 0)];
            }
            r[i] = off[i] >= 0 ? v : make_float4(0.f, 0.f, 0.f, 0.f);
// ... 82 lines not shown
```

ctrlhair_amd/csrc/sean_model.cpp:

```cpp
#include "sean_model.h"

#include <cmath>
#include <cstring>
#include <type_traits>

#include "ace_sparse.h"
#include "conv_ace_sparse.h"
#include "conv_mfma.h"
#include "conv_sh16.h"
#include "conv_pw.h"
#include "conv_wino.h"
#include "conv_wino4v.h"
#include "kernels.h"
#include "sh16.h"

namespace chk {

size_t SeanModel::noise_floats(int S) const {
    size_t n = 0;
    for (const auto& b : blocks) {
        const size_t r = (size_t)S / b.res_div;
        n += r * r * (b.learned ? 3 : 2);
    }
    return n;
// ... 549 lines not shown
            m.ev_int.assign(n_aces, nullptr);
            for (auto& e : m.ev_x)
                if (hipEventCreateWithFlags(&e, hipEventDisableTiming) != hipSuccess) return "event creation failed";
            for (auto& e : m.ev_int)
                if (hipEventCreateWithFlags(&e, hipEventDisableTiming) != hipSuccess) return "event creation failed";
            m.claim_pool = static_cast<unsigned*>(B.dalloc((size_t)SeanModel::CLAIM_SLOTS * SeanModel::CLAIM_WORDS * sizeof(unsigned)));
        }
        m.ahead_limit = limit;
        if (limit <= 0) return "";
        m.ahead_full = m.overlap_on || (long long)mb * ms * ms <= limit;
        if (!m.overlap_on && (hipStreamCreateWithFlags(&m.side, hipStreamNonBlocking) != hipSuccess || hipEventCreateWithFlags(&m.ev_fork, hipEventDisableTiming) != hipSuccess))
            return "side stream creation failed";
        m.ev_join.assign(n_aces, nullptr);
        m.actv_ahead.assign(n_aces, nullptr);
        m.lut_ahead.assign(n_aces, nullptr);
        for (auto& e : m.ev_join)
            if (hipEventCreateWithFlags(&e, hipEventDisableTiming) != hipSuccess) return "event creation failed";
        for_each_ace(m.blocks, [&](const AceW& a) {
            const size_t r = (size_t)ms / a.res_div;
            if (m.ahead_full) m.actv_ahead[a.index] = B.falloc((size_t)mb * r * (r + 64) * (HID + 20));
            if (a.styled) m.lut_ahead[a.index] = B.falloc(npad() * 18 * a.C);
        });
        m.splitk_side = B.falloc((size_t)m.splitk_cap);
        return "";
    }

    size_t npad() const { return (((size_t)mb * (LABEL_NC + 1) + 31) / 32) * 32; }
    std::string arena() {
        const size_t MB = mb, S = ms;
        for (int k = 1; k <= 5; ++k) {
            const size_t r = S >> k;
            m.lab_r[k] = static_cast<uint8_t*>(B.dalloc(MB * r * r));
        }
        size_t nf = m.noise_floats(ms);
        m.noise_ws = static_cast<float*>(B.dalloc(MB * nf * 4));
        m.mu_img = static_cast<float*>(B.dalloc((size_t)STYLE * npad() * 4));
        if (m.mu_img) (void)hipMemset(m.mu_img, 0, (size_t)STYLE * npad() * 4);
        style_projections();
        style_lut_groups();
        size_t lutmax = 0, h0max = 0, midmax = 0, outmax = 0;
        for (const auto& b : m.blocks) {
            const size_t r = S / b.res_div, px = MB * r * r;
            if (b.styled) lutmax = std::max(lutmax, npad() * 18 * b.fin);
            h0max = std::max(h0max, px * b.fin);
            midmax = std::max(midmax, px * b.fmid);
            outmax = std::max(outmax, px * b.fout);
        }
        outmax = std::max(outmax, (size_t)MB * 16 * m.ngf * (S / 32) * (S / 32));
        if (m.has_zencoder) {
            h0max = std::max(h0max, MB * S * S * 128);
            midmax = std::max(midmax, MB * S * S * (opt.use_sh16 ? 64 : 16));
        }
        m.lut = static_cast<float*>(B.dalloc(lutmax * 4));
        m.actv = static_cast<float*>(B.dalloc(MB * S * S * HID * 4));
        m.h0 = static_cast<float*>(B.dalloc(h0max * 4));
        m.hs = static_cast<float*>(B.dalloc(h0max * 4));
        m.dx = static_cast<float*>(B.dalloc(midmax * 4));
        m.h1 = static_cast<float*>(B.dalloc(midmax * 4));
        m.xs = static_cast<float*>(B.dalloc(outmax * 4));
        m.xa = static_cast<float*>(B.dalloc(outmax * 4));
        m.xb = static_cast<float*>(B.dalloc(outmax * 4));
        return "";
    }
    void style_projections() {
        const int n_aces = m.n_aces;
        m.fcmu_batched = opt.use_sh16 ? mb * (LABEL_NC + 1) > 64 : mb * LABEL_NC > 64;
        if (!m.fcmu_batched) return;
        m.mu_stride = (long long)STYLE * npad();
        m.mu_all = static_cast<float*>(B.dalloc((size_t)n_aces * m.mu_stride * 4));
        if (m.mu_all) (void)hipMemset(m.mu_all, 0, (size_t)n_aces * m.mu_stride * 4);
        std::vector<const float*> wp(n_aces, nullptr), bp(n_aces, nullptr);
        for_each_ace(m.blocks, [&](const AceW& a) {
            if (a.styled) { wp[a.index] = a.fcmu_w; bp[a.index] = a.fcmu_b; }
        });
        m.fcmu_w_ptrs = static_cast<const float**>(B.dalloc(n_aces * sizeof(float*)));
        m.fcmu_b_ptrs = static_cast<const float**>(B.dalloc(n_aces * sizeof(float*)));
        if (m.fcmu_w_ptrs && m.fcmu_b_ptrs) {
            (void)hipMemcpy(m.fcmu_w_ptrs, wp.data(), n_aces * sizeof(float*), hipMemcpyHostToDevice);
            (void)hipMemcpy(m.fcmu_b_ptrs, bp.data(), n_aces * sizeof(float*), hipMemcpyHostToDevice);
        }
    }
    void style_lut_groups() {
        m.lut_groups = nullptr;
        m.lut_ngroups = m.lut_group_tiles = 0;
        m.lut_group_rows = 0.0;
        if (!(m.fcmu_batched && !opt.use_sh16 && opt.lut_grouped)) return;
        if (m.lut_ahead.empty()) m.lut_ahead.assign(m.n_aces, nullptr);
        std::vector<PwGroup> g;
        bool ok = true;
        for_each_ace(m.blocks, [&](const AceW& a) {
            if (a.styled && (!a.lut_wt || (18 * a.C) % 128)) ok = false;
        });
        for_each_ace(m.blocks, [&](const AceW& a) {
            if (!ok || !a.styled) return;
            if (!m.lut_ahead[a.index]) m.lut_ahead[a.index] = B.falloc(npad() * 18 * a.C);
            PwGroup e{};
            e.in = a.lut_wt;
            e.wpk = m.mu_all + (size_t)a.index * m.mu_stride;
            e.out = m.lut_ahead[a.index];
            e.HW = 18 * a.C;
            e.start = m.lut_group_tiles;
            if (!e.out) { ok = false; return; }
            m.lut_group_tiles += e.HW / 128;
            m.lut_group_rows += e.HW;
            g.push_back(e);
        });
        if (ok && !g.empty()) {
            m.lut_groups = B.dalloc(g.size() * sizeof(PwGroup));
            if (m.lut_groups) (void)hipMemcpy(m.lut_groups, g.data(), g.size() * sizeof(PwGroup), hipMemcpyHostToDevice);
            m.lut_ngroups = (int)g.size();
        }
    }

    std::string wino_levels() {
        for (int k = 0; k < 6; ++k) {
            m.wq_level[k] = SeanModel::WinoLevel();
            m.actv_lvl[k] = nullptr;
        }
        m.pad_state.clear();
        m.wsty = m.wsty4 = nullptr;
        if (!(opt.wino && !opt.use_sh16)) return "";
        size_t wsty_max = 0, wsty4_max = 0;
        int lvl_planes[6] = {0, 0, 0, 0, 0, 0};
        for_each_ace(m.blocks, [&](const AceW& a) {
            if (!a.spade_wino) return;
            const int k = level_of(a.res_div), r = ms >> k;
            if (r < 32 || r % 32) return;
            SeanModel::WinoLevel& L = m.wq_level[k];
            if (!L.qlist) wino_level_lists(L, r);
            const int nrt = (a.C + 15) / 16;
            bool have = false;
            for (const auto& w : L.works) have = have || w.nrt == nrt;
            if (!have) {
                SeanModel::WinoWork w;
                w.nrt = nrt;
                w.work = static_cast<unsigned*>(B.dalloc(((size_t)L.cap_tiles * 4 + mb) * ((nrt + 1) / 2) * sizeof(unsigned)));
                w.total = static_cast<int*>(B.dalloc(8 * sizeof(int)));
                L.works.push_back(w);
            }
            lvl_planes[k] = std::max(lvl_planes[k], a.styled ? HID + 20 : HID);
            if (a.styled) wsty_max = std::max(wsty_max, (size_t)mb * nrt * 5 * 2048);
            if (a.styled && a.spade_wino4) wsty4_max = std::max(wsty4_max, (size_t)mb * nrt * 6 * wino4::ADW);
        });
        if (wsty_max) m.wsty = B.falloc(wsty_max);
        m.patchbuf = nullptr;
        m.patch_cap_chunks = 0;
        if (opt.patch && opt.wino_gather && mb <= 32) {
            m.patch_cap_chunks = 32 * mb;
            m.patchbuf = B.falloc((size_t)m.patch_cap_chunks * (HID + 20) * 1024);
        }
        if (wsty4_max) m.wsty4 = B.falloc(wsty4_max);
        wino4v_buffer();
        for (int k = 0; k < 6; ++k)
            if (m.wq_level[k].qlist) {
                const size_t r = (size_t)ms >> k;
                m.actv_lvl[k] = B.falloc((size_t)mb * r * wino_apitch((int)r) * lvl_planes[k]);
            }
        return "";
    }
    void wino_level_lists(SeanModel::WinoLevel& L, int r) {
        const bool gather = opt.wino_gather && mb <= 32 && (r / 2) * (r / 2) <= 2048 * 64;
        L.TH = gather ? 16 : opt.wino_tile_h(r);
        L.cap_tiles = mb * (r / 32) * (r / L.TH);
        L.qlist = static_cast<uint8_t*>(B.dalloc((size_t)L.cap_tiles * 8 * L.TH));
        L.qcnt = static_cast<int*>(B.dalloc((size_t)L.cap_tiles * sizeof(int)));
        L.pcnt = static_cast<int*>(B.dalloc((size_t)L.cap_tiles * sizeof(int)));
        if (gather) {
            L.gq_cap = (r / 2) * (r / 2);
            L.gq = static_cast<unsigned*>(B.dalloc((size_t)mb * L.gq_cap * sizeof(unsigned)));
            L.gq_n = static_cast<int*>(B.dalloc(32 * sizeof(int)));
            L.qoff = static_cast<int*>(B.dalloc((size_t)L.cap_tiles * sizeof(int)));
            L.chunk_base = static_cast<int*>(B.dalloc(34 * sizeof(int)));
            L.patch_mode = static_cast<int*>(B.dalloc(sizeof(int)));
        }
    }
    void wino4v_buffer() {
        m.vbuf = nullptr;
        m.vbuf_bytes = 0;
        if (!(opt.wino >= 2 && opt.wino4v)) return;
        size_t need = 0;
        auto level_r = [&](int res_div) {
            const int r = ms >> level_of(res_div);
            return (r < 32 || r % 32 || r > 64) ? 0 : r;
        };
        for (const auto& b : m.blocks)
            for (const ConvW* c : {&b.conv_0, &b.conv_1})
                if (const int r = level_r(b.res_div))
                    if (c->wino4 && wino4v_pays(c->Cout, r)) need = std::max(need, wino4v_bytes(mb, r, r, c->Cin / 4));
        for_each_ace(m.blocks, [&](const AceW& a) {
            if (const int r = level_r(a.res_div))
                if (m.ace_route_shape(a, r) == AceRoute::F4 && wino4v_pays(2 * a.C, r)) need = std::max(need, wino4v_bytes(mb, r, r, 38));
        });
        if (m.z14_wino4 && (ms / 2) % 32 == 0 && wino4v_bytes(mb, ms / 2, ms / 2, 64) <= ((size_t)5 << 29)) need = std::max(need, wino4v_bytes(mb, ms / 2, ms / 2, 64));
        if (need) {
            m.vbuf = static_cast<float*>(B.dalloc(need));
            m.vbuf_bytes = need;
        }
    }

    std::string sparse_levels() {
        m.prof_stats_cap = 16384;
        m.prof_stats_used = 0;
        m.prof_stats = static_cast<int*>(B.dalloc((size_t)m.prof_stats_cap * 4 * sizeof(int)));
        for (int k = 0; k < 6; ++k) {
            m.sp_level[k][0] = m.sp_level[k][1] = SparseLevel();
            m.sp_work[k].clear();
        }
        m.gtab = m.gtab_side = nullptr;
        if (!opt.sparse) return "";
        int cmax = 0;
        for_each_ace(m.blocks, [&](const AceW& a) {
            const int k = level_of(a.res_div), r = ms >> k;
            if (r < opt.sparse_min_r || r < 32) return;
            const int mt = (a.C + 31) / 32;
            const int th = opt.use_sh16 ? 16 : opt.sparse_tile_h(mt, r);
            SparseLevel& L = m.sp_level[k][th == 16 ? 1 : 0];
            if (!L.u5) {
                L.TH = th;
                L.cap_tiles = mb * ((r + 31) / 32) * ((r + L.TH - 1) / L.TH);
                L.u5 = static_cast<uint8_t*>(B.dalloc((size_t)mb * r * r));
                L.e16 = (opt.edge && (opt.use_sh16 || opt.wino) && r >= 128) ? static_cast<uint16_t*>(B.dalloc((size_t)mb * r * r * sizeof(uint16_t))) : nullptr;
                L.need = static_cast<uint8_t*>(B.dalloc((size_t)mb * r * r));
                L.list = static_cast<uint16_t*>(B.dalloc((size_t)L.cap_tiles * 32 * L.TH * sizeof(uint16_t)));
                L.cnt = static_cast<int*>(B.dalloc((size_t)L.cap_tiles * sizeof(int)));
            }
            bool have = false;
            for (const auto& w : m.sp_work[k]) have = have || w.mtiles == mt;
            if (!have) {
                SparseWork w;
                w.mtiles = mt;
                w.TH = L.TH;
                w.mode = opt.use_sh16 ? (opt.sh16_compact ? (opt.sh16_compact >= 2 ? 2 : 3) : 1) : 0;
                w.cap = (long long)L.cap_tiles * (opt.use_sh16 ? mt : sparse_max_tasks(L.TH, mt));
                w.work = static_cast<unsigned*>(B.dalloc((size_t)w.cap * sizeof(unsigned)));
// ... 284 lines not shown
            } else {
                check(wino_quad_lists(o.S ? o.S->u5 : nullptr, L.qlist, L.qcnt, L.pcnt, B, r, r, L.TH, st), "wino_quad_lists");
                if (L.gq) check(wino_gather_lists(L.qlist, L.qcnt, L.qoff, L.gq, L.gq_n, L.gq_cap, B, r, r, st), "wino_gather_lists");
                if (L.gq && L.chunk_base) check(wino_chunk_base(L.gq_n, B, m.patchbuf ? m.patch_cap_chunks : 0, L.chunk_base, L.patch_mode, st), "wino_chunk_base");
            }
            ls.wq_done = true;
        }
        bool done = false;
        for (int d : ls.wwork_done) done = done || d == nrt;
        if (!done) {
            if (geo && ls.geo_slot >= 0 && geo->nw < WinoGeoGroup::MAX_W) {
                WinoGeoGroup::Work& w = geo->w[geo->nw++];
                w.level = ls.geo_slot;
                w.nrt = nrt;
                w.work = p.W->work;
                w.total = p.W->total;
            } else {
                if (geo && ls.geo_slot >= 0) geo_flush();
                if (L.gq) check(wino_gather_worklist(L.gq_n, L.pcnt, B, ntiles / B, nrt, p.W->work, p.W->total, st), "wino_gather_worklist");
                else check(wino_ace_worklist(L.qcnt, L.pcnt, ntiles, nrt, p.W->work, p.W->total, st), "wino_ace_worklist");
            }
            ls.wwork_done.push_back(nrt);
        }
        return o;
    }
    WinoGeoGroup* geo = nullptr;
    void geo_flush() {
        if (!geo) return;
        if (geo->nl) check(wino_geometry_grouped(*geo, st), "level geometry (grouped)");
        geo->nl = geo->nw = 0;
        for (LevelState& s : lvl) s.geo_slot = -1;
    }
    const uint8_t* level_u5(const AcePlan& p) const {
        if (!m.opt.sparse || p.r < m.opt.sparse_min_r) return nullptr;
        for (int ti = 1; ti >= 0; --ti)
            if (m.sp_level[p.k][ti].u5 && lvl[p.k].done[ti]) return m.sp_level[p.k][ti].u5;
        return nullptr;
    }
    std::vector<AcePlan> plans;
    void plan_aces(const uint8_t* labfull) {
        plans.assign(m.n_aces, AcePlan());
        for_each_ace(m.blocks, [&](const AceW& a) {
            AcePlan& p = plans[a.index];
            p.a = &a;
            p.k = level_of(a.res_div);
            p.r = S / a.res_div;
            p.lab = a.res_div == 1 ? labfull : m.lab_r[p.k];
            p.route = m.ace_route(a, p.r, B);
            p.abuf = (p.wino() && m.actv_lvl[p.k]) ? m.actv_lvl[p.k] : m.actv;
            p.kout = a.styled ? HID + 20 : HID;
            p.ahead.lut_ns = 18 * a.C;
            if (p.wino()) {
                p.L = &m.wq_level[p.k];
                p.W = m.wino_work(a, p.r);
                if (p.route == AceRoute::WinoQuads && p.L->gq && mode.ahead != SeanModel::ChunkMode::FULL && m.patchbuf && !mode.overlap) p.patch = p.L;
                return;
            }
            p.sw = m.sparse_work(a, p.r);
            if (p.route != AceRoute::Sparse) return;
            p.SL = &m.sp_level[p.k][p.sw->TH == 16 ? 1 : 0];
            p.compact = m.opt.use_sh16 && p.sw->mode >= 2;
            if (mode.ahead == SeanModel::ChunkMode::FULL) return;
            if (m.opt.use_sh16 ? p.compact : (m.opt.dbg & 131072) != 0) p.need = p.SL->need;
            if (m.opt.use_sh16 && !p.compact) p.tile_cnt = p.SL->cnt;
        });
    }
    void prepass() {
        for (const AcePlan& p : plans)
            if (p.route == AceRoute::WinoQuads) (void)wino_prepare(p);
    }

    AcePrep build_lut(const AcePlan& pl, const float* codes, hipStream_t s, float* lut_buf, float* splitk, bool prof) {
        const AceW& a = *pl.a;
        AcePrep q;
        q.lut_ns = 18 * a.C;
        if (!a.styled) return q;
        q.lut = lut_buf;
        const int bs = m.opt.use_sh16 ? LABEL_NC + 1 : LABEL_NC;
        const int N = B * bs, npad = ((N + 31) / 32) * 32;
        q.lut_bs = bs;
        const double fl = 2.0 * 18 * a.C * STYLE * N, by = 4.0 * (18.0 * a.C * STYLE + (double)STYLE * N + 18.0 * a.C * N);
        auto tm = [&](auto launch) { prof ? timed(2, fl, by, launch) : launch(); };
        if (a.lut_rows && N <= 64 && !m.opt.batch_inv) {
            check(fc_mu(codes, a.fcmu_w, a.fcmu_b, m.mu_img, B, npad, s, m.mu_img, 0, bs), "fc_mu");
            tm([&] { check(lut_gemv_mfma(m.mu_img, a.lut_rows, lut_buf, N, 18 * a.C, s), "lut gemv"); });
            return q;
        }
        ConvParams p{};
        p.in = m.mu_img;
        p.wpk = a.lut_wpk;
        p.out = lut_buf;
        p.B = 1;
        p.Cin = STYLE;
        p.H = npad / 32;
        p.W = 32;
        p.Mrows = 18 * a.C;
        p.pad = -1;
        if (m.opt.use_sh16) {
            unsigned* mu_slot = m.amax_slots + 2 * a.index + 1;
            if (m.fcmu_batched) {
                p.in = m.mu_all + (size_t)a.index * m.mu_stride;
            } else {
                for (int pass = 0; pass < 2; ++pass)
                    check(fc_mu(codes, a.fcmu_w, a.fcmu_b, m.mu_img, B, npad, s, nullptr, 1, bs, SH16_ACT_SCALE, mu_slot, pass, m.opt.terms == 2), "fc_mu");
            }
            p.act = ACT_NONE;
            p.terms = m.opt.terms;
            p.wscale = a.lut_wscale;
            p.in_scale_inv = 1.f / SH16_ACT_SCALE;
            p.in_amax = mu_slot;
            p.out_mul = a.out_scale;
            p.partial = splitk;
            p.partial_cap = m.splitk_cap;
            tm([&] { check(conv_sh16_plain(p, 1, s), "lut gemm"); });
            q.lut_rs = npad;
            q.lut_ns = 4;
        } else {
            if (m.fcmu_batched && (N > 64 || m.opt.batch_inv)) p.in = m.mu_all + (size_t)a.index * m.mu_stride;
            else check(fc_mu(codes, a.fcmu_w, a.fcmu_b, m.mu_img, B, npad, s), "fc_mu");
            p.npix_valid = N;
            tm([&] { check(conv_nhwc1x1(p, s), "lut gemm"); });
        }
        return q;
    }
    void zero_pads(float* buf, int r, int kout, hipStream_t s) {
        const long long geo = ((long long)r << 20) | ((long long)kout << 8) | 1;
        auto it = m.pad_state.find(buf);
        if (it != m.pad_state.end() && it->second == geo) return;
        check(hipMemsetAsync(buf, 0, (size_t)m.max_batch * kout * r * wino_apitch(r) * sizeof(float), s), "hidden activations: zero pads");
        m.pad_state[buf] = geo;
    }
    void build_hidden(const AcePlan& pl, hipStream_t s, float* actv_buf) {
        const AceW& a = *pl.a;
        const int r = pl.r, kout = pl.kout;
        const uint8_t* lab = pl.lab;
        if (!pl.wino()) m.pad_state.erase(actv_buf);
        if (m.opt.use_sh16)
            check(onehot_conv3x3_sh16(lab, a.actv_table, a.actv_bias, actv_buf, B, r, r, HID, 1, a.actv_scale, s, m.opt.terms == 2, pl.need, pl.tile_cnt,
                                      (m.opt.dbg & 33554432) ? 1 : 0), "mlp_shared");
        else if (pl.wino()) {
            zero_pads(actv_buf, r, kout, s);
            const uint8_t* u5 = (pl.route == AceRoute::WinoQuads && m.opt.hidden_wq) ? level_u5(pl) : nullptr;
            const SeanModel::WinoLevel* PL = pl.patch;
            const bool pm = PL && PL->gq && PL->patch_mode && m.patchbuf;
            if (pm && mode.prologue && PL->chunk_base) {
                check(spade_hidden_level(lab, u5, PL->gq, PL->gq_n, PL->gq_cap, PL->chunk_base, PL->patch_mode, a.actv_table,
                                         a.actv_bias, actv_buf, m.patchbuf, B, r, r, kout, a.styled ? 1 : 0, wino_apitch(r), WINO_AXOFF, s),
                      "mlp_shared (planes or pre-gathered patches)");
                return;
            }
            check(spade_hidden_wq(lab, u5, a.actv_table, a.actv_bias, actv_buf, B, r, r, kout, a.styled ? 1 : 0, s,
                                  wino_apitch(r), WINO_AXOFF, pm ? PL->patch_mode : nullptr), "mlp_shared (boundary-quad patches)");
            if (pm) check(spade_hidden_patch(lab, PL->gq, PL->gq_n, PL->gq_cap, PL->chunk_base, PL->patch_mode, a.actv_table, a.actv_bias, m.patchbuf,
                                             B, r, r, kout, s), "mlp_shared (pre-gathered patches)");
        } else
            check(onehot_conv3x3(lab, a.actv_table, a.actv_bias, actv_buf, B, r, r, HID, 1, s, 0, pl.need), "mlp_shared");
    }

    void prepare_all_ahead(const float* codes) {
        const bool full = mode.ahead == SeanModel::ChunkMode::FULL;
        check(hipEventRecord(m.ev_fork, st), "fork");
        check(hipStreamWaitEvent(m.side, m.ev_fork, 0), "fork wait");
        for (AcePlan& p : plans) {
            const AceW& a = *p.a;
            if (!full && !a.styled) continue;
            if (!(mode.grouped && a.styled)) p.ahead = build_lut(p, codes, m.side, m.lut_ahead[a.index], m.splitk_side, false);
            p.ahead.actv = m.actv_ahead[a.index];
            if (full) build_hidden(p, m.side, m.actv_ahead[a.index]);
            check(hipEventRecord(m.ev_join[a.index], m.side), "join record");
        }
    }

    void luts_grouped() {
        const int N = B * LABEL_NC;
        PwParams q{};
        q.Cin = STYLE;
        q.Cout = N;
        q.groups = static_cast<const PwGroup*>(m.lut_groups);
        q.ngroups = m.lut_ngroups;
        const int nrg = ((N + 31) / 32 + 3) / 4;
        timed(2, 2.0 * m.lut_group_rows * STYLE * N, 4.0 * (m.lut_group_rows * STYLE + m.lut_group_rows * N + (double)m.lut_ngroups * STYLE * N),
              [&] { check(conv_pw_grouped(q, m.lut_group_tiles * nrg, st), "style LUTs (grouped GEMM)"); });
        for (AcePlan& p : plans)
            if (p.a->styled) p.ahead.lut = m.lut_ahead[p.a->index];
    }

    void prologue() {
        HiddenGroup hg{};
        AceTableGroup tg{};
        StylePackGroup sg{};
        WinoGeoGroup gg{};
        hg.B = tg.B = sg.B = gg.B = B;
        geo = &gg;
        tg.lut_rs = 1;
        tg.lut_bs = LABEL_NC;
        tg.lut_mul = 1.f;
        for (AcePlan& p : plans) {
            const AceW& a = *p.a;
            const int r = p.r;
            if (p.route == AceRoute::F4) {
                float* buf = m.pro_actv[a.index];
                if (!buf || hg.n >= HiddenGroup::MAX) continue;
                zero_pads(buf, r, p.kout, st);
                HiddenGroup::Entry& e = hg.e[hg.n++];
                e.lab = p.lab;
                e.u5 = nullptr;
                e.table = a.actv_table;
                e.bias = a.actv_bias;
                e.out = buf;
                e.H = e.W = r;
                e.kout = p.kout;
                e.onehot = a.styled ? 1 : 0;
                e.pitch = wino_apitch(r);
                e.xoff = WINO_AXOFF;
                p.pre_actv = buf;
                continue;
            }
            if (p.route != AceRoute::WinoQuads) continue;
            const WinoPrep wp = wino_prepare(p);
            if (a.styled && !mode.grouped) continue;
            const float* lut = a.styled ? p.ahead.lut : nullptr;
            if (a.styled && !lut) continue;
            const bool p6 = wp.edges && a.styled;
            if (wp.S && m.pro_gtab[a.index] && (!p6 || m.pro_p6[a.index]) && tg.n < AceTableGroup::MAX) {
                AceTableGroup::Entry& e = tg.e[tg.n++];
                e.bias_g = a.bias_g;
                e.bias_b = a.bias_b;
                e.gconst = a.gconst;
                e.lut = lut;
                e.gtab = m.pro_gtab[a.index];
                e.p6 = p6 ? m.pro_p6[a.index] : nullptr;
                e.C = a.C;
                p.pre_gtab = e.gtab;
                p.pre_p6 = e.p6;
            }
            if (a.styled && m.pro_wsty[a.index] && sg.n < StylePackGroup::MAX) {
                StylePackGroup::Entry& e = sg.e[sg.n++];
                e.lut = lut;
                e.wsty = m.pro_wsty[a.index];
                e.C = a.C;
                p.pre_wsty = e.wsty;
            }
        }
        geo_flush();
        geo = nullptr;
        check(spade_hidden_wq_grouped(hg, st), "mlp_shared (grouped, F(4x4)-route ACEs)");
        check(ace_tables_grouped(tg, st), "ace tables (grouped)");
        check(wino_style_pack_grouped(sg, st), "wino_style_pack (grouped)");
    }

    void ace(const AceW& a, const float* codes, const float* noise, size_t nf, size_t noff, const float* x, int x_up, int act, float* hout) {
        const AcePlan& p = plans[a.index];
        const AceIO io{noise + noff, (long long)nf, x, x_up, act, hout};
        const WinoPrep wp = p.route == AceRoute::WinoQuads ? wino_prepare(p) : WinoPrep();
        if (p.sw) sparse_prepare(p);
        const AcePrep q = operands(p, codes);
        switch (p.route) {
            case AceRoute::F4: return ace_f4(p, q, io);
            case AceRoute::WinoQuads: return ace_wino(p, wp, q, io);
            case AceRoute::Sparse: return ace_sparse(p, q, io);
            case AceRoute::TinySplitK: return ace_tiny(p, q, io);
            case AceRoute::Dense: return ace_dense(p, q, io);
        }
    }
    AcePrep operands(const AcePlan& p, const float* codes) {
        const AceW& a = *p.a;
        AcePrep q;
        if (mode.ahead == SeanModel::ChunkMode::FULL) {
            q = p.ahead;
            check(hipStreamWaitEvent(st, m.ev_join[a.index], 0), "join wait");
        } else {
            const bool lut_made = a.styled && (mode.grouped || mode.ahead == SeanModel::ChunkMode::LUTS);
            if (!lut_made) q = build_lut(p, codes, st, m.lut, m.splitk_ws, true);
            if (!p.pre_actv) build_hidden(p, st, p.abuf);
            if (lut_made) q = p.ahead;
            q.actv = p.abuf;
            if (lut_made && !mode.grouped) check(hipStreamWaitEvent(st, m.ev_join[a.index], 0), "join wait");
        }
        if (p.pre_actv) q.actv = p.pre_actv;
        return q;
    }
    template <class P>
    void fill_mod(P& t, const AcePlan& p, const AceIO& io) {
        const AceW& a = *p.a;
        t.x = io.x;
        t.x_up = io.x_up;
        t.act = io.act;
        t.out = io.out;
        t.B = B;
        t.C = a.C;
        t.H = t.W = p.r;
        t.bn_a = a.bn_a;
        t.bn_d = a.bn_d;
        t.nv = a.nv;
        t.noise = io.noise;
        t.noise_bstride = io.nf;
        if constexpr (!std::is_same<P, AceInteriorParams>::value) {
            t.bias_g = a.bias_g;
            t.bias_b = a.bias_b;
        }
    }
    AceInteriorParams interior_params(const AcePlan& p, const AceIO& io, const SparseLevel& L) {
        AceInteriorParams ip{};
        fill_mod(ip, p, io);
        ip.u5 = L.u5;
        ip.cnt = L.cnt;
        ip.gtab = m.gtab;
        return ip;
    }
    void interior_edges(AceInteriorParams& ip, const AcePlan& p, const AcePrep& q, const SparseLevel& L) {
        ip.e16 = L.e16;
        ip.etab = p.a->edge_tab;
        ip.p6 = (p.a->styled && q.lut) ? m.p6 : nullptr;
    }
    double dense_flops(const AcePlan& p) const { return 2.0 * 2 * p.a->C * HID * 9 * ((double)B * p.r * p.r); }

    void ace_f4(const AcePlan& p, const AcePrep& q, const AceIO& io) {
        const AceW& a = *p.a;
        const int r = p.r;
        const double npix = (double)B * r * r;
        Wino4AceParams w{};
        fill_mod(w, p, io);
        w.actv = q.actv;
        w.wpk = a.spade_wino4;
        w.wsty = (a.styled && q.lut) ? m.wsty4 : nullptr;
        const int nks = w.wsty ? 38 : 32, ktot = 4 * nks;
        next_flops_exec = 2.0 * 32.0 * ((a.C + 15) / 16) * ktot * 36.0 * npix / 16.0;
        Wino4vPackParams vp;
        const bool vroute = m.wino4v_route(wino4v_pays(2 * a.C, r), q.actv, B, r, p.kout, nks, vp, true);
        timed(1, dense_flops(p), 4.0 * (npix * p.kout + npix * a.C / (io.x_up ? 4.0 : 1.0) + npix * a.C), [&] {
            if (w.wsty) check(wino4_style_pack(q.lut, m.wsty4, B, a.C, st), "wino4_style_pack");
            if (vroute) {
                check(wino4v_pack(vp, st), "hidden activation transform (winograd F(4x4,3x3))");
                w.v = m.vbuf;
                check(conv_wino4v_ace(w, st), "spade conv (winograd F(4x4,3x3), every tile, pre-transformed input)");
            } else
                check(conv_wino4_ace(w, st), "spade conv (winograd F(4x4,3x3), every tile)");
        });
    }
    void ace_wino(const AcePlan& p, const WinoPrep& wp, const AcePrep& q, const AceIO& io) {
        const AceW& a = *p.a;
        const int r = p.r, x_up = io.x_up;
        const double npix = (double)B * r * r;
        const double xpp = 4.0 * a.C / (x_up ? 4.0 : 1.0), opp = 4.0 * a.C;
        const int ktot = p.kout;
        if (wp.S) {
            AceInteriorParams ip = interior_params(p, io, *wp.S);
            ip.impl = r >= 128 ? 2 : 0;
            ip.groups = m.opt.int_groups;
            ip.onepass = m.opt.int_onepass;
            if (wp.edges) {
                if (!a.edge_tab || r < 128) check(hipErrorInvalidValue, "straight-edge marks on a level whose ACE has no table");
                interior_edges(ip, p, q, *wp.S);
            }
            ip.fill_min = (x_up && r < 128) ? 257 : ((r >= 128 && !(m.opt.dbg & 134217728)) ? 0 : 128);
            if (mode.overlap) {
                ip.fill_min = 257;
                ip.quad_only = 1;
                ip.gtab = m.gtab_side;
                check(hipEventRecord(m.ev_x[a.index], st), "x ready");
                check(hipStreamWaitEvent(m.side_int, m.ev_x[a.index], 0), "x ready wait");
                check(ace_gtable(a.bias_g, a.bias_b, a.gconst, q.lut, q.lut_rs, q.lut_ns, q.lut_bs, 1.f, m.gtab_side, B, a.C, m.side_int), "ace_gtable");
                check(ace_interior_f32(ip, m.side_int), "ace interior");
                check(hipEventRecord(m.ev_int[a.index], m.side_int), "interior done");
            } else {
                const bool pre = p.pre_gtab && (ip.p6 != nullptr) == (p.pre_p6 != nullptr);
                if (pre) {
                    ip.gtab = p.pre_gtab;
                    ip.p6 = p.pre_p6;
                }
                timed(3, 0.0, 0.0, SpStat{p.W->total + 4, 0.0, xpp + opp + 5.0, 4.0 * 19 * 2 * a.C * B, npix}, [&] {
                    if (!pre) {
                        check(ace_gtable(a.bias_g, a.bias_b, a.gconst, q.lut, q.lut_rs, q.lut_ns, q.lut_bs, 1.f, m.gtab, B, a.C, st), "ace_gtable");
                        if (ip.p6) check(ace_p6table(q.lut, q.lut_rs, q.lut_ns, q.lut_bs, 1.f, m.p6, B, a.C, st), "ace_p6table");
                    }
                    check(ace_interior_f32(ip, st), "ace interior");
                });
            }
        }
        const SeanModel::WinoLevel& L = *p.L;
        WinoAceParams w{};
        fill_mod(w, p, io);
        w.actv = q.actv;
        w.wpk = a.spade_wino;
        const float* pre_wsty = (a.styled && q.lut) ? p.pre_wsty : nullptr;
        w.wsty = (a.styled && q.lut) ? (pre_wsty ? pre_wsty : m.wsty) : nullptr;
        w.patch = p.patch ? m.patchbuf : nullptr;
        w.chunk_base = L.chunk_base;
        w.patch_mode = L.patch_mode;
        w.qlist = L.qlist;
        w.TH = L.TH;
        w.qcnt = L.qcnt;
        w.work = p.W->work;
        w.total = p.W->total;
        w.zero = m.zero_page;
        w.gq = L.gq;
        w.gq_n = L.gq_n;
        w.gq_cap = L.gq_cap;
        w.claim = w.gq ? next_claim() : nullptr;
        timed(1, dense_flops(p), 0.0, SpStat{p.W->total + 4, 2.0 * 32 * 16 * 16 * ktot, 4.0 * ktot + xpp + opp, 4.0 * 2.0 * a.C * ktot * 16, npix}, [&] {
            if (w.wsty && !pre_wsty) check(wino_style_pack(q.lut, m.wsty, B, a.C, st), "wino_style_pack");
            check(conv_wino_ace(w, st), "spade conv (winograd, boundary quads)");
        });
        if (mode.overlap && wp.S) check(hipStreamWaitEvent(st, m.ev_int[a.index], 0), "interior done wait");
    }
    ConvParams ace_conv_params(const AcePlan& pl, const AcePrep& q, const AceIO& io) {
        const AceW& a = *pl.a;
        ConvParams p{};
        fill_mod(p, pl, io);
        p.in = q.actv;
        p.wpk = a.spade_wpk;
        p.Cin = HID;
        p.Mrows = 2 * a.C;
        p.lab = pl.lab;
// ... 112 lines not shown
        p.wpk = w.wpk;
        p.out = out;
        p.B = B;
        p.Cin = w.Cin;
        p.H = r;
        p.W = r;
        p.Mrows = w.Cout;
        p.bias = w.bias;
        p.res = res;
        p.res_up = res_up;
        p.act = ACT_NONE;
        p.pad = -1;
        p.dbg = m.opt.dbg;
        p.terms = m.opt.terms;
        p.wscale = w.wscale;
        p.in_scale_inv = 1.f / prod.out_scale;
        p.partial = m.opt.batch_inv ? nullptr : m.splitk_ws;
        p.partial_cap = m.splitk_cap;
        p.mtiles_hint_small = (((w.Cout + 63) / 64) * (((long long)B * r * r + 511) / 512) < 192) ? 1 : 0;
        const double npix = (double)B * r * r, k2 = w.KS * w.KS, cin2 = w2 ? w2->Cin : 0;
        if (m.opt.wino >= 2 && !m.opt.use_sh16 && w.wino4 && w.KS == 3 && !w2 && wino4_supported(r, r, w.Cin) &&
            (!use_wino(w, r) || m.opt.wino4_force || m.opt.batch_inv || wino4_pays((long long)B * (r / 32) * (r / 32) * ((w.Cout + 31) / 32), m.num_cus))) {
            Wino4Params q{};
            q.in = in;
            q.wpk = w.wino4;
            q.out = out;
            q.B = B;
            q.Cin = w.Cin;
            q.Cout = w.Cout;
            q.H = r;
            q.W = r;
            q.bias = w.bias;
            q.res = res;
            q.res_up = res_up;
            q.wpk_split = w.wino4s;
            q.split = m.opt.wino4_split;
            next_flops_exec = 2.0 * w.Cout * w.Cin * 36.0 * npix / 16.0;
            Wino4vPackParams vp;
            const bool vroute = m.wino4v_route(wino4v_pays(w.Cout, r), in, B, r, w.Cin, w.Cin / 4, vp);
            timed(0, 2.0 * w.Cout * w.Cin * 9.0 * npix,
                  4.0 * (npix * w.Cin + npix * w.Cout * (res ? 2.0 : 1.0) + (double)w.Cout * w.Cin * 36.0), [&] {
                      if (vroute) {
                          check(wino4v_pack(vp, st), "conv input transform (winograd F(4x4,3x3))");
                          q.v = m.vbuf;
                          check(conv_wino4v_plain(q, st), "conv (winograd F(4x4,3x3), pre-transformed input)");
                      } else
                          check(conv_wino4_plain(q, st), "conv (winograd F(4x4,3x3))");
                  });
            return;
        }
        if (use_wino(w, r) && !w2 && !(r == 16 && res_up)) {
            WinoParams q{};
            q.in = in;
            q.wpk = w.wino;
            q.out = out;
            q.B = B;
            q.Cin = w.Cin;
            q.Cout = w.Cout;
            q.H = r;
            q.W = r;
            q.bias = w.bias;
            q.res = res;
            q.res_up = res_up;
            q.act = ACT_NONE;
            q.zero = m.zero_page;
            q.claim = next_claim();
            q.partial = m.opt.batch_inv ? nullptr : m.splitk_ws;
            q.partial_cap = m.splitk_cap;
            next_flops_exec = 2.0 * w.Cout * w.Cin * 16.0 * npix / 4.0;
            timed(0, 2.0 * w.Cout * w.Cin * 9.0 * npix,
                  4.0 * (npix * w.Cin + npix * w.Cout * (res ? 2.0 : 1.0) + (double)w.Cout * w.Cin * 16.0),
                  [&] { check(conv_wino_plain(q, st), "conv (winograd)"); });
            return;
        }
        if (m.opt.wino && !m.opt.use_sh16 && w.pw && w.KS == 1 && !w2 && !res && !w.bias && pw_supported(w.Cin, w.Cout, r * r)) {
            PwParams q{};
            q.in = in;
            q.wpk = w.pw;
            q.out = out;
            q.B = B;
            q.Cin = w.Cin;
            q.Cout = w.Cout;
            q.HW = r * r;
            timed(0, 2.0 * w.Cout * w.Cin * npix, 4.0 * (npix * w.Cin + npix * w.Cout + (double)w.Cout * w.Cin),
                  [&] { check(conv_pw(q, st), "conv 1x1"); });
            return;
        }
        timed(0, 2.0 * w.Cout * (w.Cin * k2 + cin2) * npix,
              4.0 * (npix * (w.Cin + cin2) + npix * w.Cout * (res ? 2.0 : 1.0) + (double)w.Cout * (w.Cin * k2 + cin2)), [&] {
                  if (m.opt.use_sh16) check(conv_sh16_plain(p, w.KS, st), "conv");
                  else check(w.KS == 3 ? conv_plain3(p, st) : conv_plain1(p, st), "conv");
              });
    }
};

}

static uint64_t chunk_seed(uint64_t seed, int bo) { return seed + 0x632BE59BD9B4E019ull * (uint64_t)(bo + 1); }

std::string SeanModel::draw_noise(uint64_t seed, float* out, int Btot, int S, hipStream_t st) {
    if (blocks.empty()) return "model not finalized";
    if (S % 32 != 0 || S < 32 || S > max_size) return "S must be a multiple of 32 and <= max_size";
    const size_t nf = noise_floats(S);
    for (int bo = 0; bo < Btot; bo += max_batch) {
        const int B = std::min(max_batch, Btot - bo);
        if (gen_noise(out + (size_t)bo * nf, (long long)B * nf, chunk_seed(seed, bo), st) != hipSuccess) return "gen_noise failed";
    }
    return "";
}

std::string SeanModel::generate(const uint8_t* labels, const float* codes, const float* noise, uint64_t seed,
                                float* out, int Btot, int S, hipStream_t st) {
    if (blocks.empty()) return "model not finalized";
    if (S % 32 != 0 || S < 32 || S > max_size) return "S must be a multiple of 32 and <= max_size";
    if (Btot < 1) return "B must be >= 1";
    const size_t nf = noise_floats(S);
    hipStream_t st_user = st;
    if (overlap_on) {
        if (hipEventRecord(ev_in, st_user) != hipSuccess || hipStreamWaitEvent(main_i, ev_in, 0) != hipSuccess) return "overlap mode: fork failed";
        st = main_i;
    }
    auto join = [&](const std::string& e) {
        if (overlap_on && (hipEventRecord(ev_out, main_i) != hipSuccess || hipStreamWaitEvent(st_user, ev_out, 0) != hipSuccess) && e.empty())
            return std::string("overlap mode: join failed");
        return e;
    };
    for (int bo = 0; bo < Btot; bo += max_batch) {
        const int B = std::min(max_batch, Btot - bo);
        const uint8_t* lab = labels + (size_t)bo * S * S;
        Runner R(*this, st, B, S, lab);
        const ChunkMode& mode = R.mode;
        if (claim_pool) R.check(hipMemsetAsync(claim_pool, 0, (size_t)CLAIM_SLOTS * CLAIM_WORDS * sizeof(unsigned), st), "claim counters");
        const float* cd = codes + (size_t)bo * LABEL_NC * STYLE;
        const float* nz;
        if (noise) {
            nz = noise + (size_t)bo * nf;
        } else {
            R.check(gen_noise(noise_ws, (long long)B * nf, chunk_seed(seed, bo), st), "gen_noise");
            nz = noise_ws;
        }
        for (int k = 1; k <= 5; ++k) R.check(label_downsample(lab, lab_r[k], B, S, S >> k, st), "label_downsample");
        if (opt.use_sh16) R.check(hipMemsetAsync(amax_slots, 0, 64 * sizeof(unsigned), st), "amax slots");
        if (mode.project_all) {
            R.check(fc_mu_batched(cd, fcmu_w_ptrs, fcmu_b_ptrs, mu_all, mu_stride, n_aces, B, ((B * LABEL_NC + 31) / 32) * 32, LABEL_NC, 1.f,
                                  nullptr, 0, 0, st, mode.grouped ? 2 : 0), "fc_mu (all ACEs)");
            if (mode.grouped) R.luts_grouped();
        } else if (fcmu_batched && opt.use_sh16) {
            const int npad_c = ((B * (LABEL_NC + 1) + 31) / 32) * 32;
            for (int pass = 0; pass < 2; ++pass)
                R.check(fc_mu_batched(cd, fcmu_w_ptrs, fcmu_b_ptrs, mu_all, mu_stride, n_aces, B, npad_c, LABEL_NC + 1, SH16_ACT_SCALE,
                                      amax_slots, pass, opt.terms == 2, st), "fc_mu (all ACEs)");
        }
        if (mode.prepass) R.prepass();
        if (mode.ahead != ChunkMode::NONE) R.prepare_all_ahead(cd);
        if (mode.prologue) R.prologue();

        const int sw = S / 32;
        float* x = xa;
        float* y = xb;
        R.check(onehot_conv3x3(lab_r[5], fc_table, fc_bias, x, B, sw, sw, 16 * ngf, 0, st, opt.use_sh16 ? 1 : 0), "fc");
        R.tap_c4("fc", x, 16 * ngf, (size_t)sw * sw);
        size_t noff = 0;
        for (const auto& b : blocks) {
            const int r = S / b.res_div;
            const size_t rr = (size_t)r * r;
            const int up = b.up_before ? 1 : 0;
            const float* xsrc = x;
            const float* shortcut;
            int sc_up;
            bool fuse_s = false;
            if (b.learned) {
                R.ace(b.ace_s, cd, nz, nf, noff, xsrc, up, ACT_NONE, hs);
                noff += rr;
                R.tap_sh16(b.name + ".hs", hs, b.fin, rr, b.ace_s);
                fuse_s = R.can_fuse_1x1(b.conv_1, r) && !taps.count(b.name + ".xs") && !R.use_wino(b.conv_1, r);
                if (!fuse_s) {
                    R.conv(b.conv_s, hs, b.ace_s, xs, r, nullptr, 0);
                    R.tap_c4(b.name + ".xs", xs, b.fout, rr);
                }
                shortcut = fuse_s ? nullptr : xs;
                sc_up = 0;
            } else {
                shortcut = xsrc;
                sc_up = up;
            }
            R.ace(b.ace_0, cd, nz, nf, noff, xsrc, up, ACT_LRELU, h0);
            noff += rr;
            R.tap_sh16(b.name + ".h0", h0, b.fin, rr, b.ace_0);
            R.conv(b.conv_0, h0, b.ace_0, dx, r, nullptr, 0);
            R.tap_c4(b.name + ".dx", dx, b.fmid, rr);
            R.ace(b.ace_1, cd, nz, nf, noff, dx, 0, ACT_LRELU, h1);
            noff += rr;
            R.tap_sh16(b.name + ".h1", h1, b.fmid, rr, b.ace_1);
            R.conv(b.conv_1, h1, b.ace_1, y, r, shortcut, sc_up, fuse_s ? &b.conv_s : nullptr, fuse_s ? hs : nullptr, fuse_s ? &b.ace_s : nullptr);
            R.tap_c4(b.name, y, b.fout, rr);
            std::swap(x, y);
        }
        R.check(conv_img_tanh(x, img_w, img_b, out + (size_t)bo * 3 * S * S, B, ngf, S, S, st, opt.use_sh16 ? 1 : 0, img_w4), "conv_img");
        if (!R.err.empty()) return join(R.err);
    }
    return join("");
}

std::string SeanModel::encode(const float* img, const uint8_t* labels, float* codes_out, int Btot, int S,
                              hipStream_t st, int phase) {
    if (blocks.empty() || !has_zencoder) return "Zencoder weights not loaded/finalized";
    if (S % 32 != 0 || S < 32 || S > max_size) return "S must be a multiple of 32 and <= max_size";
    if (phase != 0 && Btot > max_batch) return "split encode: B must not exceed max_batch";
    if (phase == 1) { enc_pending_B = Btot; enc_pending_S = S; }
    if (phase == 2 && (enc_pending_B != Btot || enc_pending_S != S)) return "split encode: no matching ch_sean_encode_features call";
    if (phase == 2) enc_pending_B = 0;
    for (int bo = 0; bo < Btot; bo += max_batch) {
        const int B = std::min(max_batch, Btot - bo);
        std::string err;
        auto ck = [&](hipError_t e, const char* what) {
            if (e != hipSuccess && err.empty()) err = std::string(what) + ": " + hipGetErrorString(e);
        };
        const float* x = img + (size_t)bo * 3 * S * S;
        ConvOpts refl;
        refl.pad_mode = PAD_REFLECT;
        ConvOpts zero;
        ConvOpts zins;
        zins.in_mode = IN_UP2_ZEROINS;
        ConvOpts last = refl;
        last.act = ACT_TANH;
        const int h2 = S / 2, h4 = S / 4;
        const bool f16path = opt.use_sh16 && h4 * h4 >= 4096;
        bool in4_done = false;
        if (phase != 2) {
        ck(conv3x3_c3_reflect(x, z1_w, z1.bias, hs, B, 32, S, S, st), "zenc conv1");
        if (f16path) {
            auto s2d = [&](const ConvLayer& L, const float* in, float* out, int hin, const char* what) {
                ConvParams q{};
                q.in = in;
                q.wpk = L.sh_wpk;
                q.wscale = L.sh_wscale;
                q.in_scale_inv = 1.f / instnorm_sh16_scale(hin * hin);
                q.out = out;
                q.B = B;
                q.Cin = L.Cin;
                q.s2d_cr = L.s2d_cr;
                q.s2d_phase0 = L.s2d_phase0;
                q.H = hin / 2;
                q.W = hin / 2;
                q.Mrows = L.Cout;
                q.bias = L.bias;
                q.act = ACT_NONE;
                ck(conv_sh16_s2d(q, L.KS, st), what);
            };
            ck(instnorm_act(hs, B * 32, S * S, 1e-5f, ACT_LRELU, st, h0, 32, splitk_ws), "zenc in1");
            s2d(z4_s2d, h0, dx, S, "zenc conv2 (f16x3)");
            ck(instnorm_c4_to_sh16(dx, B, 64, h2 * h2, 1e-5f, ACT_LRELU, h1, st, splitk_ws), "zenc in2");
            s2d(z7_s2d, h1, hs, h2, "zenc conv3 (f16x3)");
            ck(instnorm_c4_to_sh16(hs, B, 128, h4 * h4, 1e-5f, ACT_LRELU, dx, st, splitk_ws), "zenc in3");
        } else {
            ck(instnorm_act(hs, B * 32, S * S, 1e-5f, ACT_LRELU, st), "zenc in1");
            ck(run_conv(z4, hs, dx, B, S, S, zero, st), "zenc conv2");
            ck(instnorm_act(dx, B * 64, h2 * h2, 1e-5f, ACT_LRELU, st), "zenc in2");
            ck(run_conv(z7, dx, h1, B, h2, h2, zero, st), "zenc conv3");
        }
        if (f16path) {
            ConvParams t{};
            t.in = dx;
            t.out = hs;
            t.B = B;
            t.Cin = 128;
            t.bias = z10.bias;
            t.in_scale_inv = 1.f / instnorm_sh16_scale(h4 * h4);
            t.act = ACT_NONE;
            if (opt.dbg & 16384) {
                t.wpk = z10_sh;
                t.wscale = z10_ws;
                t.H = h2;
                t.W = h2;
                t.Mrows = 256;
                t.in_mode = IN_UP2_ZEROINS;
                ck(conv_sh16_plain(t, 3, st), "zenc convT (f16x3)");
            } else {
                t.wpk = z10_d2s;
                t.wscale = z10_d2s_ws;
                t.H = h4;
                t.W = h4;
                t.Mrows = 1024;
                ck(conv_sh16_d2s(t, st), "zenc convT (f16x3, depth-to-space)");
            }
            ck(instnorm_c4_to_sh16(hs, B, 256, h2 * h2, 1e-5f, ACT_LRELU, h1, st, splitk_ws), "zenc in4");
        } else {
            ck(instnorm_act(h1, B * 128, h4 * h4, 1e-5f, ACT_LRELU, st), "zenc in3");
            const long long hw4 = (long long)h4 * h4;
            if (z10_pw[3] && !opt.use_sh16 && !opt.batch_inv && pw_supported(128, 256, (int)hw4) && (h4 & 3) == 0 && (long long)B * hw4 >= 16384 && vbuf &&
                (size_t)B * (512 + 4 * 256) * hw4 * sizeof(float) <= vbuf_bytes) {
                float *xs = vbuf, *tph = vbuf + (size_t)B * 512 * hw4;
                ck(convt_shift4(h1, xs, B, 128, h4, h4, st), "zenc convT shifted views");
                static const int first[4] = {1, 0, 1, 0}, cnt[4] = {1, 2, 2, 4};
                for (int ph = 0; ph < 4; ++ph) {
                    PwParams q{};
                    q.in = xs + (size_t)first[ph] * 128 * hw4;
                    q.in_bs = 512 * hw4;
                    q.wpk = z10_pw[ph];
                    q.out = tph + (size_t)ph * B * 256 * hw4;
                    q.B = B;
                    q.Cin = cnt[ph] * 128;
                    q.Cout = 256;
                    q.HW = (int)hw4;
                    ck(conv_pw(q, st), "zenc convT (phase GEMM)");
                }
                ck(instnorm_act_d2s(tph, z10.bias, hs, B, 256, h4, h4, 1e-5f, ACT_LRELU, st), "zenc in4 (depth-to-space)");
                in4_done = true;
            } else if (z10_wino && !opt.use_sh16 && wino_supported(h4, h4, 128)) {
                WinoParams q{};
                q.in = h1;
                q.wpk = z10_wino;
                q.out = hs;
                q.B = B;
                q.Cin = 128;
                q.Cout = 1024;
                q.H = h4;
                q.W = h4;
                q.bias = z10.bias;
                q.act = ACT_NONE;
                q.d2s = 1;
                q.zero = zero_page;
                ck(conv_wino_plain(q, st), "zenc convT (winograd phase convs)");
            } else
                ck(run_conv(z10, h1, hs, B, h4, h4, zins, st), "zenc convT");
            if (opt.use_sh16) ck(instnorm_act(hs, B * 256, h2 * h2, 1e-5f, ACT_LRELU, st, h1, 256), "zenc in4");
        }
        if (opt.use_sh16) {
            ConvParams p{};
            p.in = h1;
            p.wpk = z14_sh;
            p.out = h0;
            p.B = B;
            p.Cin = 256;
            p.H = h2;
            p.W = h2;
            p.Mrows = 512;
            p.bias = z14.bias;
            p.wscale = z14_ws;
            p.in_scale_inv = 1.f / instnorm_sh16_scale(h2 * h2);
            p.act = ACT_TANH;
            p.pad_mode = PAD_REFLECT;
            ck(conv_sh16_plain(p, 3, st), "zenc conv5 (f16x3)");
        } else {
            if (!in4_done) ck(instnorm_act(hs, B * 256, h2 * h2, 1e-5f, ACT_LRELU, st), "zenc in4");
            if (z14_wino4 && wino4_supported(h2, h2, 256) && (opt.wino4_force || opt.batch_inv || wino4_pays((long long)B * (h2 / 32) * (h2 / 32) * 16, num_cus))) {
                Wino4Params q{};
                q.in = hs;
                q.wpk = z14_wino4;
                q.out = h0;
                q.B = B;
                q.Cin = 256;
                q.Cout = 512;
                q.H = h2;
                q.W = h2;
                q.bias = z14.bias;
                q.act = ACT_TANH;
                q.reflect = 1;
                q.wpk_split = z14_wino4s;
                q.split = opt.wino4_split;
                Wino4vPackParams vp;
                if (wino4v_route(true, hs, B, h2, 256, 64, vp, false, true)) {
                    ck(wino4v_pack(vp, st), "zenc conv5 input transform");
                    q.v = vbuf;
                    ck(conv_wino4v_plain(q, st), "zenc conv5 (winograd F(4x4,3x3), pre-transformed input)");
                } else
                    ck(conv_wino4_plain(q, st), "zenc conv5 (winograd F(4x4,3x3))");
            } else if (z14_wino && wino_supported(h2, h2, 256)) {
                WinoParams q{};
                q.in = hs;
                q.wpk = z14_wino;
                q.out = h0;
                q.B = B;
                q.Cin = 256;
                q.Cout = 512;
                q.H = h2;
                q.W = h2;
                q.bias = z14.bias;
                q.act = ACT_TANH;
                q.reflect = 1;
                q.zero = zero_page;
                ck(conv_wino_plain(q, st), "zenc conv5 (winograd)");
            } else
                ck(run_conv(z14, hs, h0, B, h2, h2, last, st), "zenc conv5");
        }
        }
        if (phase == 1) {
// ... 89 lines not shown
```

ctrlhair_amd/csrc/sean_model.h:

```cpp
#pragma once
#include <hip/hip_runtime.h>
#include <stdint.h>

#include <map>
#include <string>
#include <vector>

#include "ace_sparse.h"
#include "net_common.h"

namespace chk {
struct Wino4vPackParams;

struct ConvW {
    float* wpk = nullptr;
    float* bias = nullptr;
    float* wscale = nullptr;
    float* wino = nullptr;
    float* wino4 = nullptr;
    float* wino4s = nullptr;
    float* pw = nullptr;
    int Cout = 0, Cin = 0, KS = 0;
};

struct AceW {
    std::string name;
    int C = 0, res_div = 1, index = 0;
    bool styled = false;
    float* spade_wpk = nullptr;
    float *bias_g = nullptr, *bias_b = nullptr;
    float *bn_a = nullptr, *bn_d = nullptr, *nv = nullptr;
    float *actv_table = nullptr, *actv_bias = nullptr;
    float *fcmu_w = nullptr, *fcmu_b = nullptr;
    float* lut_wpk = nullptr;
    float* lut_rows = nullptr;
    float* lut_wt = nullptr;
    float *spade_wscale = nullptr, *lut_wscale = nullptr;
    float out_scale = 8.f;
    float actv_scale = 1.f;
    float* spade_wino = nullptr;
    float* edge_tab = nullptr;
    float* spade_wino4 = nullptr;
    float* gconst = nullptr;
};

struct BlockW {
    std::string name;
    int fin = 0, fout = 0, fmid = 0, res_div = 1;
    bool up_before = false, styled = false, learned = false;
    ConvW conv_0, conv_1, conv_s;
    AceW ace_0, ace_1, ace_s;
};

struct ProfRec {
    hipEvent_t e0, e1;
    int kind;
    double flops, bytes;
    double flops_exec = -1.0;
    const int* sp_stat = nullptr;
    double sp_flops_unit = 0.0;
    double sp_bytes_px = 0.0, sp_bytes_fixed = 0.0, sp_npix = 0.0;
};

template <class Blocks, class F>
void for_each_ace(Blocks& blocks, F fn) {
    for (auto& b : blocks)
        for (auto* a : {b.learned ? &b.ace_s : nullptr, &b.ace_0, &b.ace_1})
            if (a) fn(*a);
}
inline int level_of(int res_div) {
    int k = 0;
    while ((1 << k) < res_div) ++k;
    return k;
}

enum class AceRoute {
    F4,
    WinoQuads,
    Sparse,
    TinySplitK,
    Dense
};

struct SeanOptions {
    bool use_sh16 = false;
    int terms = 3;
    int wino = 2;
    int lut_grouped = 1;
    int prologue = 1;
    int overlap = 0;
    int wino4_force = 0;
    int patch = 1;
    int convt_gemm = 1;
    int edge = 1;
    int frame = 1;
    int int_groups = 0;
    int int_onepass = 1;
    int batch_inv = 0;
    int wino4v = 1;
    int wino4_split = -1;
    int wino4_ace_max_r = 64;
    int hidden_wq = 1;
    int wino_gather = 1;
    int wino_th = 0;
    int wino_tile_h(int r) const { return (wino_th == 16 || wino_th == 32) ? (r % wino_th ? 16 : wino_th) : ((r >= 512 || r == 128) ? 32 : 16); }
    int sparse = 1;
    int sh16_compact = 1;
    int sparse_th = 0;
    int sparse_tile_h(int mtiles, int r) const {
        return sparse_th == 8 || sparse_th == 16 ? sparse_th : ((mtiles <= 2 || r >= 512) ? 16 : 8);
    }
    int sparse_min_r = 64;
    long long ahead_pixels = -1;
    int dbg = 0;
    int dbg_sel = 16;
};

struct SeanModel {
    SeanOptions opt;
    int ngf = 0, max_batch = 0, max_size = 0;
    int num_cus = 256;
    std::vector<void*> allocs;

    std::vector<BlockW> blocks;
    int n_aces = 0;
    float *fc_table = nullptr, *fc_bias = nullptr;
    float *img_w = nullptr, *img_b = nullptr;
    float* img_w4 = nullptr;
    bool has_zencoder = false;
    float* z1_w = nullptr;
    ConvLayer z1, z4, z7, z10, z14;
    float *z14_sh = nullptr, *z10_sh = nullptr;
    float* z10_wino = nullptr;
    float* z10_pw[4] = {};
    float* z14_wino = nullptr;
    float* z14_wino4s = nullptr;
    float* z14_wino4 = nullptr;
    float *z14_ws = nullptr, *z10_ws = nullptr;
    float *z10_d2s = nullptr, *z10_d2s_ws = nullptr;
    ConvLayer z4_s2d, z7_s2d;

    float* gb_small = nullptr;
    long long gb_small_cap = 0;
    float* splitk_ws = nullptr;
    long long splitk_cap = 0;
    uint8_t* lab_r[6] = {nullptr, nullptr, nullptr, nullptr, nullptr, nullptr};
    unsigned* amax_slots = nullptr;
    float* zero_page = nullptr;
    float *noise_ws = nullptr, *mu_img = nullptr, *lut = nullptr, *actv = nullptr;
    bool fcmu_batched = false;
    float* mu_all = nullptr;
    long long mu_stride = 0;
    const float** fcmu_w_ptrs = nullptr;
    const float** fcmu_b_ptrs = nullptr;
    float *h0 = nullptr, *hs = nullptr, *dx = nullptr, *h1 = nullptr, *xs = nullptr, *xa = nullptr, *xb = nullptr;
    int enc_pending_B = 0, enc_pending_S = 0;

    hipStream_t side = nullptr;
    hipEvent_t ev_fork = nullptr;
    std::vector<hipEvent_t> ev_join;
    std::vector<float*> actv_ahead, lut_ahead;
    void* lut_groups = nullptr;
    int lut_ngroups = 0, lut_group_tiles = 0;
    double lut_group_rows = 0.0;
    bool ahead_full = false;
    long long ahead_limit = 0;
    float* splitk_side = nullptr;
    bool overlap_on = false;
    hipStream_t main_i = nullptr, side_int = nullptr;
    hipEvent_t ev_in = nullptr, ev_out = nullptr;
    std::vector<hipEvent_t> ev_x, ev_int;
    unsigned* claim_pool = nullptr;
    static constexpr int CLAIM_SLOTS = 96, CLAIM_WORDS = 1024;

    struct WinoWork { int nrt = 0; unsigned* work = nullptr; int* total = nullptr; };
    struct WinoLevel {
        uint8_t* qlist = nullptr; int* qcnt = nullptr; int* pcnt = nullptr; int cap_tiles = 0, TH = 16; std::vector<WinoWork> works;
        unsigned* gq = nullptr; int* gq_n = nullptr; int* qoff = nullptr; int gq_cap = 0;
        int* chunk_base = nullptr;
        int* patch_mode = nullptr;
    };
    WinoLevel wq_level[6];
    float* actv_lvl[6] = {nullptr, nullptr, nullptr, nullptr, nullptr, nullptr};
    std::map<const float*, long long> pad_state;
    float* patchbuf = nullptr;
    int patch_cap_chunks = 0;
    float* wsty = nullptr;
    float* wsty4 = nullptr;
    float* vbuf = nullptr;
    size_t vbuf_bytes = 0;
    bool wino4v_route(bool pays, const float* in, int Bn, int r, int K, int nks, Wino4vPackParams& vp, bool padded = false, bool reflect = false) const;
    const WinoWork* wino_work(const AceW& a, int r) const;
    const SparseWork* sparse_work(const AceW& a, int r) const;
    AceRoute ace_route_shape(const AceW& a, int r) const;
    AceRoute ace_route(const AceW& a, int r, int B) const;
    struct ChunkMode {
        bool project_all = false, grouped = false;
        enum Ahead { NONE, LUTS, FULL } ahead = NONE;
        bool prepass = false, overlap = false;
        bool prologue = false;
    };
    ChunkMode chunk_mode(int B, int S) const;
    bool pro_on = false;
    std::vector<float*> pro_actv, pro_gtab, pro_p6, pro_wsty;
    size_t pro_bytes = 0;

    SparseLevel sp_level[6][2];
    std::vector<SparseWork> sp_work[6];
    float* gtab = nullptr;
    float* gtab_side = nullptr;
    float* p6 = nullptr;

    bool prof_on = false;
    std::vector<ProfRec> prof;
    std::vector<hipEvent_t> ev_pool;
    int* prof_stats = nullptr;
    int prof_stats_cap = 0, prof_stats_used = 0;
    std::map<std::string, float*> taps;

    size_t noise_floats(int S) const;
    std::string build(const TensorStore& ts, int max_batch, int max_size);
    std::string generate(const uint8_t* labels, const float* codes, const float* noise, uint64_t seed, float* out,
                         int B, int S, hipStream_t stream);
    std::string draw_noise(uint64_t seed, float* out, int B, int S, hipStream_t stream);
    std::string encode(const float* img, const uint8_t* labels, float* codes_out, int B, int S, hipStream_t stream, int phase = 0);
    void destroy();
};

}
```

Measured before the change: 572.7 images/s.

## Add wide-tile pointwise GEMM kernel and row-based Winograd style packing

Adds a pw_conv_wide kernel in which each wave computes a 2x2 grid of 32x32 MFMA tiles (two row tiles by two pixel groups), so A and B fragments are reused across more accumulators. It is selected by default for 1x1 convs, the grouped style-LUT GEMM and the convT phase GEMM. Tasks whose row group lies past Cout now skip their MFMAs and stores in both the wide and the old kernel. The Winograd F(4x4) style pack gains a rows variant that writes only the valid units over a buffer zeroed once, and fc_mu gets a transposed template path. The wider kernel uses more registers and LDS, and the grouped path needs HW to be a multiple of 256.

```diff
diff --git a/ctrlhair_amd/csrc/ch_api.cpp b/ctrlhair_amd/csrc/ch_api.cpp
--- a/ctrlhair_amd/csrc/ch_api.cpp
+++ b/ctrlhair_amd/csrc/ch_api.cpp
@@ -749,6 +749,7 @@
     {"sean.frame", BY_SEAN, BOOL, 0, 0, SEAN_FIELD(frame)},
     {"sean.int_groups", NEVER, CLAMP, 0, MAXI, SEAN_FIELD(int_groups)},
     {"sean.int_onepass", NEVER, BOOL, 0, 0, SEAN_FIELD(int_onepass)},
+    {"sean.pw_wide", NEVER, BOOL, 0, 0, SEAN_FIELD(pw_wide)},
     {"sean.batch_invariant", NEVER, BOOL, 0, 0, SEAN_FIELD(batch_inv)},
     {"sean.wino4v", BY_SEAN, BOOL, 0, 0, SEAN_FIELD(wino4v)},
     {"sean.wino4_split", BY_SEAN, CLAMP, -1, 1, SEAN_FIELD(wino4_split)},
diff --git a/ctrlhair_amd/csrc/conv_inst_wino.hip b/ctrlhair_amd/csrc/conv_inst_wino.hip
--- a/ctrlhair_amd/csrc/conv_inst_wino.hip
+++ b/ctrlhair_amd/csrc/conv_inst_wino.hip
@@ -116,17 +116,37 @@
     hipLaunchKernelGGL(pw_conv_kernel<RT>, dim3(grid), dim3(512), Cfg::LDS_BYTES, s, p);
     return hipGetLastError();
 }
+template <int RP>
+static hipError_t launch_pw_wide(PwParams p, hipStream_t s) {
+    using Cfg = PwWideCfg<RP>;
+    static bool d0[64] = {};
+    hipError_t e = wino_attr(pw_conv_wide_kernel<RP>, Cfg::LDS_BYTES, d0);
+    if (e != hipSuccess) return e;
+    const int nrt = (p.Cout + 31) / 32;
+    p.nrg = (nrt + Cfg::RTB - 1) / Cfg::RTB;
+    p.npt = p.HW / Cfg::PXB;
+    p.ntasks = p.B * p.npt * p.nrg;
+    p.nst = p.Cin / 16;
+    const int grid = p.ntasks < wino_num_cus() ? p.ntasks : wino_num_cus();
+    hipLaunchKernelGGL(pw_conv_wide_kernel<RP>, dim3(grid), dim3(512), Cfg::LDS_BYTES, s, p);
+    return hipGetLastError();
+}
 hipError_t conv_pw(PwParams p, hipStream_t s) {
     if (!pw_supported(p.Cin, p.Cout, p.HW)) return hipErrorInvalidValue;
     p.groups = nullptr;
     p.ngroups = 0;
+    const int rp = pw_wide_rule(p.wide, p.Cout, p.HW);
+    if (rp) return rp == 2 ? launch_pw_wide<2>(p, s) : launch_pw_wide<1>(p, s);
     return (p.Cout + 31) / 32 >= 4 ? launch_pw<4>(p, s) : launch_pw<2>(p, s);
 }
 hipError_t conv_pw_grouped(PwParams p, int ntasks, hipStream_t s) {
     using Cfg = PwCfg<4>;
+    using Wide = PwWideCfg<2>;
     if (p.Cin % 16 || p.Cout < 1 || !p.groups || p.ngroups < 1 || ntasks < 1) return hipErrorInvalidValue;
-    static bool d0[64] = {};
-    hipError_t e = wino_attr(pw_conv_kernel<4>, Cfg::LDS_BYTES, d0);
+    const bool wide = p.wide && p.Cout > 64;
+    if (wide && ntasks % (Wide::PXB / 128)) return hipErrorInvalidValue;
+    static bool d0[64] = {}, d1[64] = {};
+    hipError_t e = wide ? wino_attr(pw_conv_wide_kernel<2>, Wide::LDS_BYTES, d1) : wino_attr(pw_conv_kernel<4>, Cfg::LDS_BYTES, d0);
     if (e != hipSuccess) return e;
     p.in = p.wpk = nullptr;
     p.out = nullptr;
@@ -134,10 +154,11 @@
     p.HW = 0;
     p.nrg = ((p.Cout + 31) / 32 + 3) / 4;
     p.npt = 0;
-    p.ntasks = ntasks;
+    p.ntasks = wide ? ntasks / (Wide::PXB / 128) : ntasks;
     p.nst = p.Cin / 16;
-    const int grid = ntasks < wino_num_cus() ? ntasks : wino_num_cus();
-    hipLaunchKernelGGL(pw_conv_kernel<4>, dim3(grid), dim3(512), Cfg::LDS_BYTES, s, p);
+    const int grid = p.ntasks < wino_num_cus() ? p.ntasks : wino_num_cus();
+    if (wide) hipLaunchKernelGGL(pw_conv_wide_kernel<2>, dim3(grid), dim3(512), Wide::LDS_BYTES, s, p);
+    else hipLaunchKernelGGL(pw_conv_kernel<4>, dim3(grid), dim3(512), Cfg::LDS_BYTES, s, p);
     return hipGetLastError();
 }
 
diff --git a/ctrlhair_amd/csrc/conv_inst_wino4.hip b/ctrlhair_amd/csrc/conv_inst_wino4.hip
--- a/ctrlhair_amd/csrc/conv_inst_wino4.hip
+++ b/ctrlhair_amd/csrc/conv_inst_wino4.hip
@@ -63,6 +63,9 @@
     return hipGetLastError();
 }
 
+__device__ __forceinline__ float wino4_dot3(float a0, float b0, float a1, float b1, float a2, float b2) {
+    return __builtin_fmaf(a2, b2, __builtin_fmaf(a0, b0, a1 * b1));
+}
 __global__ __launch_bounds__(256) void wino4_style_pack_kernel(const float* __restrict__ lut, float* __restrict__ wsty, int B, int C, int nrt) {
     const long long n = (long long)B * nrt * 6 * 1152;
     const long long i = blockIdx.x * 256LL + threadIdx.x;
@@ -87,17 +90,54 @@
             const int xi = 4 * idx + e - 36 * m, ii = xi / 6, jj = xi % 6;
             float r[3];
 #pragma unroll
-            for (int q = 0; q < 3; ++q) r[q] = Gm[ii][0] * g[0][q] + Gm[ii][1] * g[1][q] + Gm[ii][2] * g[2][q];
-            u[e] = r[0] * Gm[jj][0] + r[1] * Gm[jj][1] + r[2] * Gm[jj][2];
+            for (int q = 0; q < 3; ++q) r[q] = wino4_dot3(Gm[ii][0], g[0][q], Gm[ii][1], g[1][q], Gm[ii][2], g[2][q]);
+            u[e] = wino4_dot3(r[0], Gm[jj][0], r[1], Gm[jj][1], r[2], Gm[jj][2]);
         }
         o = make_float4(u[0], u[1], u[2], u[3]);
     }
     reinterpret_cast<float4*>(wsty)[i] = o;
 }
-hipError_t wino4_style_pack(const float* lut, float* wsty, int B, int C, hipStream_t s) {
+__global__ __launch_bounds__(256) void wino4_style_pack_rows_kernel(const float* __restrict__ lut, float* __restrict__ wsty, int B, int C, int nrt) {
+    const long long n = (long long)B * nrt * 5 * 128;
+    const long long i = blockIdx.x * 256LL + threadIdx.x;
+    if (i >= n) return;
+    const int lane = (int)(i & 63), m = (int)((i >> 6) & 1), s = (int)((i >> 7) % 5);
+    const int rt = (int)((i / 640) % nrt), b = (int)(i / (640LL * nrt));
+    const int j = 4 * s + (lane >> 4);
+    if (j >= 19) return;
+    float4* dst = reinterpret_cast<float4*>(wsty) + (((long long)b * nrt + rt) * 6 + s) * 1152 + 9 * m * 64 + lane;
+    int ch, beta;
+    wino4_ace_row(rt * 32 + m * 16 + (lane & 15), ch, beta);
+    if (ch >= C) {
+#pragma unroll
+        for (int k = 0; k < 9; ++k) dst[k * 64] = make_float4(0.f, 0.f, 0.f, 0.f);
+        return;
+    }
+    const float* P = lut + ((long long)(b * 19 + j) * 9) * 2 * C + beta * C + ch;
+    float g[3][3];
+#pragma unroll
+    for (int t = 0; t < 9; ++t) g[t / 3][t % 3] = P[(long long)t * 2 * C];
+    const float Gm[6][3] = {{0.25f, 0.f, 0.f}, {-1.f / 6, -1.f / 6, -1.f / 6}, {-1.f / 6, 1.f / 6, -1.f / 6},
+                            {1.f / 24, 1.f / 12, 1.f / 6}, {1.f / 24, -1.f / 12, 1.f / 6}, {0.f, 0.f, 1.f}};
+#pragma unroll
+    for (int k = 0; k < 9; ++k) {
+        float u[4];
+#pragma unroll
+        for (int e = 0; e < 4; ++e) {
+            const int xi = 4 * k + e, ii = xi / 6, jj = xi % 6;
+            float r[3];
+#pragma unroll
+            for (int q = 0; q < 3; ++q) r[q] = wino4_dot3(Gm[ii][0], g[0][q], Gm[ii][1], g[1][q], Gm[ii][2], g[2][q]);
+            u[e] = wino4_dot3(r[0], Gm[jj][0], r[1], Gm[jj][1], r[2], Gm[jj][2]);
+        }
+        dst[k * 64] = make_float4(u[0], u[1], u[2], u[3]);
+    }
+}
+hipError_t wino4_style_pack(const float* lut, float* wsty, int B, int C, hipStream_t s, int rows) {
     const int nrt = (C + 15) / 16;
-    const long long n = (long long)B * nrt * 6 * 1152;
-    hipLaunchKernelGGL(wino4_style_pack_kernel, dim3((unsigned)((n + 255) / 256)), dim3(256), 0, s, lut, wsty, B, C, nrt);
+    const long long n = rows ? (long long)B * nrt * 5 * 128 : (long long)B * nrt * 6 * 1152;
+    if (rows) hipLaunchKernelGGL(wino4_style_pack_rows_kernel, dim3((unsigned)((n + 255) / 256)), dim3(256), 0, s, lut, wsty, B, C, nrt);
+    else hipLaunchKernelGGL(wino4_style_pack_kernel, dim3((unsigned)((n + 255) / 256)), dim3(256), 0, s, lut, wsty, B, C, nrt);
     return hipGetLastError();
 }
 
diff --git a/ctrlhair_amd/csrc/conv_pw.h b/ctrlhair_amd/csrc/conv_pw.h
--- a/ctrlhair_amd/csrc/conv_pw.h
+++ b/ctrlhair_amd/csrc/conv_pw.h
@@ -17,6 +17,7 @@
     const PwGroup* groups;
     int ngroups;
     long long in_bs;
+    int wide;
     int nrg, npt, ntasks, nst;
 };
 
@@ -142,7 +143,11 @@
     auto frag = [&](unsigned slot) { return reinterpret_cast<const float*>(smem) + (slot - lds0) / 4; };
     float4 a_lo = *reinterpret_cast<const float4*>(frag(lds0) + aoff), a_hi = *reinterpret_cast<const float4*>(frag(lds0) + aoff + 4);
     float b0 = frag(lds0)[boff], b1 = frag(lds0)[boff + 32];
+    const int nrt_all = (p.Cout + 31) / 32;
+    auto row_group = [&](int L) { return (p.groups ? L - p.groups[group_of(L)].start * p.nrg : L) % p.nrg; };
     for (int k = 0, ct = lb; k < mytasks; ++k, ct += G) {
+        const bool live = row_group(ct) * RT + rtl < nrt_all;
+        const bool live_next = k + 1 < mytasks && row_group(ct + G) * RT + rtl < nrt_all;
         for (int cs = 0; cs < nst; ++cs) {
             if (after_epi) asm volatile("s_waitcnt vmcnt(0)" ::: "memory");
             else asm volatile("s_waitcnt vmcnt(%0)" ::"n"(NLD * (NST - 3)) : "memory");
@@ -152,6 +157,16 @@
             const unsigned nslot = rslot + SB == lds0 + RING ? lds0 : rslot + SB;
             const float* sp = frag(rslot);
             const float* spn = frag(nslot);
+            if (!live) {
+                if (cs == nst - 1 && live_next) {
+                    b0 = spn[boff];
+                    b1 = spn[boff + 32];
+                    a_lo = *reinterpret_cast<const float4*>(spn + aoff);
+                    a_hi = *reinterpret_cast<const float4*>(spn + aoff + 4);
+                }
+                rslot = nslot;
+                continue;
+            }
             const float av[8] = {a_lo.x, a_lo.y, a_lo.z, a_lo.w, a_hi.x, a_hi.y, a_hi.z, a_hi.w};
 #pragma unroll
             for (int s = 0; s < 8; ++s) {
@@ -170,7 +185,7 @@
             }
             rslot = nslot;
         }
-        {
+        if (live) {
             int rg, pt, b, eHW;
             float* tout;
             if (p.groups) {
@@ -203,7 +218,202 @@
     asm volatile("s_waitcnt vmcnt(0)" ::: "memory");
 }
 
+template <int RP>
+struct PwWideCfg {
+    static constexpr int PG = 8 / RP, PXB = 64 * PG;
+    static constexpr int RTB = 2 * RP;
+    static constexpr int PDW = 16 * PXB, ADW = RTB * 512;
+    static constexpr int SDW = PDW + ADW, NST = RP == 2 ? 6 : 4;
+    static constexpr int NPD = PDW / (4 * 512);
+    static constexpr int NLD = NPD + 1;
+    static constexpr int LDS_BYTES = NST * SDW * 4 + 512 * 16;
+};
+
+template <int RP>
+__global__ __launch_bounds__(512, 1) void pw_conv_wide_kernel(const PwParams p) {
+    using Cfg = PwWideCfg<RP>;
+    constexpr int PG = Cfg::PG, PXB = Cfg::PXB, RTB = Cfg::RTB, PDW = Cfg::PDW, SDW = Cfg::SDW, NST = Cfg::NST, NPD = Cfg::NPD, NLD = Cfg::NLD;
+    constexpr int PXS = PXB / 128;
+    extern __shared__ __attribute__((aligned(16))) float smem[];
+    const int tid = threadIdx.x, lane = tid & 63;
+    const int wave = __builtin_amdgcn_readfirstlane(tid >> 6);
+    const int G = gridDim.x;
+    const int lb = xcd_remap(blockIdx.x, G);
+    if (lb >= p.ntasks) return;
+    const int mytasks = (p.ntasks - lb + G - 1) / G;
+    const int nst = p.nst;
+    constexpr unsigned SB = SDW * 4, RING = NST * SB;
+    auto group_of = [&](int L) {
+        int g = 0;
+        while (g + 1 < p.ngroups && L >= p.groups[g + 1].start / PXS * p.nrg) ++g;
+        return g;
+    };
+    const unsigned lds0 = (unsigned)(size_t)(wino_lds_void*)smem;
+
+    unsigned vp[NPD];
+    const bool a_wave = wave < RTB * 2;
+    int it = lb, is = 0;
+    wino_u32x4 d_in, d_a;
+    unsigned so_in = 0, so_a = 0;
+    int HW = p.HW;
+    const int nrt_all = (p.Cout + 31) / 32;
+    auto issue_task = [&]() {
+        int rg, pt, ib;
+        const float *tin, *twpk;
+        if (p.groups) {
+            const int g = group_of(it), local = it - p.groups[g].start / PXS * p.nrg;
+            rg = local % p.nrg;
+            pt = local / p.nrg;
+            ib = 0;
+            HW = p.groups[g].HW;
+            tin = p.groups[g].in;
+            twpk = p.groups[g].wpk;
+        } else {
+            rg = it % p.nrg;
+            pt = (it / p.nrg) % p.npt;
+            ib = it / (p.nrg * p.npt);
+            tin = p.in;
+            twpk = p.wpk;
+        }
+#pragma unroll
+        for (int i = 0; i < NPD; ++i) {
+            const int u = i * 512 + tid, ch = u / (PXB / 4), q = u - ch * (PXB / 4);
+            vp[i] = (unsigned)(ch * HW + pt * PXB + 4 * q) * 4u;
+        }
+        d_in = wino_rsrc(tin + (long long)ib * (p.in_bs ? p.in_bs : (long long)p.Cin * HW), (unsigned)p.Cin * HW * 4u);
+        const int have = nrt_all - rg * RTB < RTB ? nrt_all - rg * RTB : RTB;
+        d_a = wino_rsrc(twpk + (long long)rg * RTB * nst * 512, (unsigned)have * nst * 2048u);
+        so_in = 0;
+        so_a = 0;
+    };
+    issue_task();
+    const unsigned va_rt = a_wave ? (unsigned)((tid >> 7) * nst * 2048 + (tid & 127) * 16) : 0x80000000u;
+    unsigned islot = lds0;
+    auto issue = [&]() {
+        const unsigned wb = islot + (unsigned)wave * 1024u;
+#pragma unroll
+        for (int i = 0; i < NPD; ++i) wino_dma16(vp[i], d_in, so_in, wb + (unsigned)i * 8192u);
+        const unsigned wa = a_wave ? islot + PDW * 4u + (unsigned)wave * 1024u : lds0 + RING + (unsigned)wave * 1024u;
+        wino_dma16(va_rt, d_a, so_a, wa);
+        islot = islot + SB == lds0 + RING ? lds0 : islot + SB;
+        so_in += 64u * (unsigned)HW;
+        so_a += 2048u;
+        if (++is == nst) {
+            if (it + G < p.ntasks) {
+                it += G;
+                is = 0;
+                issue_task();
+            } else {
+                is = nst - 1;
+                so_in -= 64u * (unsigned)HW;
+                so_a -= 2048u;
+            }
+        }
+    };
+
+    f32x16 acc[2][2];
+#pragma unroll
+    for (int t = 0; t < 2; ++t)
+#pragma unroll
+        for (int n = 0; n < 2; ++n)
+#pragma unroll
+            for (int r = 0; r < 16; ++r) acc[t][n][r] = 0.f;
+    const int rp = wave / PG, pg = wave % PG;
+    const int boff = (lane >> 5) * PXB + pg * 64 + (lane & 31);
+    const int aoff = PDW + 2 * rp * 512 + lane * 8;
+
+#pragma unroll
+    for (int j = 0; j < NST - 1; ++j) issue();
+    asm volatile("s_waitcnt vmcnt(%0)" ::"n"(NLD * (NST - 3)) : "memory");
+    __syncthreads();
+    unsigned rslot = lds0;
+    bool after_epi = false;
+    auto frag = [&](unsigned slot) { return reinterpret_cast<const float*>(smem) + (slot - lds0) / 4; };
+    float4 a0_lo, a0_hi, a1_lo, a1_hi;
+    float b0, b1;
+    auto first_frags = [&](const float* f) {
+        b0 = f[boff];
+        b1 = f[boff + 32];
+        a0_lo = *reinterpret_cast<const float4*>(f + aoff);
+        a0_hi = *reinterpret_cast<const float4*>(f + aoff + 4);
+        a1_lo = *reinterpret_cast<const float4*>(f + aoff + 512);
+        a1_hi = *reinterpret_cast<const float4*>(f + aoff + 516);
+    };
+    first_frags(frag(lds0));
+    auto row_group = [&](int L) { return (p.groups ? L - p.groups[group_of(L)].start / PXS * p.nrg : L) % p.nrg; };
+    for (int k = 0, ct = lb; k < mytasks; ++k, ct += G) {
+        const bool live = row_group(ct) * RTB + 2 * rp < nrt_all;
+        const bool live_next = k + 1 < mytasks && row_group(ct + G) * RTB + 2 * rp < nrt_all;
+        for (int cs = 0; cs < nst; ++cs) {
+            if (after_epi) asm volatile("s_waitcnt vmcnt(0)" ::: "memory");
+            else asm volatile("s_waitcnt vmcnt(%0)" ::"n"(NLD * (NST - 3)) : "memory");
+            __syncthreads();
+            after_epi = false;
+            issue();
+            const unsigned nslot = rslot + SB == lds0 + RING ? lds0 : rslot + SB;
+            const float* sp = frag(rslot);
+            const float* spn = frag(nslot);
+            rslot = nslot;
+            if (!live) {
+                if (cs == nst - 1 && live_next) first_frags(spn);
+                continue;
+            }
+            const float av0[8] = {a0_lo.x, a0_lo.y, a0_lo.z, a0_lo.w, a0_hi.x, a0_hi.y, a0_hi.z, a0_hi.w};
+            const float av1[8] = {a1_lo.x, a1_lo.y, a1_lo.z, a1_lo.w, a1_hi.x, a1_hi.y, a1_hi.z, a1_hi.w};
+#pragma unroll
+            for (int s = 0; s < 8; ++s) {
+                const float c0 = b0, c1 = b1;
+                if (s < 7) {
+                    b0 = sp[boff + (2 * s + 2) * PXB];
+                    b1 = sp[boff + (2 * s + 2) * PXB + 32];
+                } else first_frags(spn);
+                acc[0][0] = __builtin_amdgcn_mfma_f32_32x32x2f32(av0[s], c0, acc[0][0], 0, 0, 0);
+                acc[1][0] = __builtin_amdgcn_mfma_f32_32x32x2f32(av1[s], c0, acc[1][0], 0, 0, 0);
+                acc[0][1] = __builtin_amdgcn_mfma_f32_32x32x2f32(av0[s], c1, acc[0][1], 0, 0, 0);
+                acc[1][1] = __builtin_amdgcn_mfma_f32_32x32x2f32(av1[s], c1, acc[1][1], 0, 0, 0);
+            }
+        }
+        if (live) {
+            int rg, pt, b, eHW;
+            float* tout;
+            if (p.groups) {
+                const int g = group_of(ct), local = ct - p.groups[g].start / PXS * p.nrg;
+                rg = local % p.nrg;
+                pt = local / p.nrg;
+                b = 0;
+                eHW = p.groups[g].HW;
+                tout = p.groups[g].out;
+            } else {
+                rg = ct % p.nrg;
+                pt = (ct / p.nrg) % p.npt;
+                b = ct / (p.nrg * p.npt);
+                eHW = p.HW;
+                tout = p.out;
+            }
+            const int row0 = (rg * RTB + 2 * rp) * 32 + 4 * (lane >> 5);
+            float* ob = tout + (long long)b * p.Cout * eHW + pt * PXB + pg * 64 + (lane & 31);
+#pragma unroll
+            for (int t = 0; t < 2; ++t)
+#pragma unroll
+                for (int n = 0; n < 2; ++n)
+#pragma unroll
+                    for (int r = 0; r < 16; ++r) {
+                        const int row = row0 + 32 * t + (r & 3) + 8 * (r >> 2);
+                        if (row < p.Cout) ob[(long long)row * eHW + n * 32] = acc[t][n][r];
+                        acc[t][n][r] = 0.f;
+                    }
+            after_epi = true;
+        }
+    }
+    asm volatile("s_waitcnt vmcnt(0)" ::: "memory");
+}
+
 inline bool pw_supported(int Cin, int Cout, int HW) { return Cin % 16 == 0 && HW % 256 == 0 && Cout >= 32; }
+inline int pw_wide_rule(int wide, int Cout, int HW) {
+    if (!wide || HW % 256 || Cout < 64) return 0;
+    if (Cout > 64) return 2;
+    return HW % 512 == 0 ? 1 : 0;
+}
 hipError_t conv_pw(PwParams p, hipStream_t s);
 inline int pw_group_tasks(int Cout, int HW) { return ((((Cout + 31) / 32) + 3) / 4) * (HW / 128); }
 hipError_t conv_pw_grouped(PwParams p, int ntasks, hipStream_t s);
diff --git a/ctrlhair_amd/csrc/conv_wino4.h b/ctrlhair_amd/csrc/conv_wino4.h
--- a/ctrlhair_amd/csrc/conv_wino4.h
+++ b/ctrlhair_amd/csrc/conv_wino4.h
@@ -641,6 +641,6 @@
 hipError_t conv_wino4_plain(Wino4Params p, hipStream_t s);
 inline bool wino4_ace_supported(int H, int W, int C) { return H % wino4::TS == 0 && W % wino4::TS == 0 && C % 2 == 0; }
 hipError_t conv_wino4_ace(Wino4AceParams p, hipStream_t s);
-hipError_t wino4_style_pack(const float* lut, float* wsty, int B, int C, hipStream_t s);
-
-}
+hipError_t wino4_style_pack(const float* lut, float* wsty, int B, int C, hipStream_t s, int rows = 0);
+
+}
diff --git a/ctrlhair_amd/csrc/kernels.h b/ctrlhair_amd/csrc/kernels.h
--- a/ctrlhair_amd/csrc/kernels.h
+++ b/ctrlhair_amd/csrc/kernels.h
@@ -46,10 +46,10 @@
                        hipStream_t s, int bf16 = 0, int single = 0);
 hipError_t fc_mu(const float* codes, const float* Wt, const float* bias, float* mu_img, int B, int Npad, hipStream_t s,
                  float* mu_rows = nullptr, int sh16 = 0, int bs = 19, float scale = 1.f, unsigned* amax = nullptr,
-                 int pass = 0, int bf16 = 0);
+                 int pass = 0, int bf16 = 0, int transposed = 1);
 hipError_t fc_mu_batched(const float* codes, const float* const* Wts, const float* const* biases, float* mu_base,
                          long long mu_stride, int n_aces, int B, int Npad, int bs, float scale, unsigned* amax_slots, int pass,
-                         int bf16, hipStream_t s, int sh16 = 1);
+                         int bf16, hipStream_t s, int sh16 = 1, int transposed = 1);
 hipError_t conv_img_tanh(const float* x, const float* w, const float* bias, float* out, int B, int Cin, int H, int W,
                          hipStream_t s, int c4 = 0, const float* w4 = nullptr);
 hipError_t c4_decode(const float* in, float* out, int B, int C, long long HW, hipStream_t s);
diff --git a/ctrlhair_amd/csrc/sean_kernels.hip b/ctrlhair_amd/csrc/sean_kernels.hip
--- a/ctrlhair_amd/csrc/sean_kernels.hip
+++ b/ctrlhair_amd/csrc/sean_kernels.hip
@@ -801,6 +801,7 @@
 
 constexpr int FCMU_BT = 8;
 
+template <bool TR>
 __device__ __forceinline__ void fc_mu_body(const float* __restrict__ codes, const float* __restrict__ Wt,
                                            const float* __restrict__ bias, float* __restrict__ mu_img, int B, int Npad,
                                            float* __restrict__ mu_rows, int sh16, int bs, float scale,
@@ -834,59 +835,94 @@
                 c1 = cr[1];
             }
 #pragma unroll
+            for (int i = 0; i < 4; ++i) {
+                float d = w[i][0].x * c0.x;
+                d = __builtin_fmaf(w[i][0].y, c0.y, d);
+                d = __builtin_fmaf(w[i][0].z, c0.z, d);
+                d = __builtin_fmaf(w[i][0].w, c0.w, d);
+                d = __builtin_fmaf(w[i][1].x, c1.x, d);
+                d = __builtin_fmaf(w[i][1].y, c1.y, d);
+                d = __builtin_fmaf(w[i][1].z, c1.z, d);
+                part[i][t] = __builtin_fmaf(w[i][1].w, c1.w, d);
+            }
+        }
+        auto emit = [&](int i, int t, float sum) {
+            const float v = sum + bias[j * 512 + o0 + i];
+            const float r = v > 0.f ? v : 0.f;
+            const int o = o0 + i, n = (bb + t) * bs + j;
+            if (bs > 19 && j == 0) {
+                const int nz = (bb + t) * bs + 19;
+                if (mu_rows) mu_rows[(long long)nz * 512 + o] = 0.f;
+                else if (sh16 == 1) {
+                    _Float16* mh = reinterpret_cast<_Float16*>(mu_img);
+                    mh[(((long long)(o >> 3) * 2 + 0) * Npad + nz) * 8 + (o & 7)] = (_Float16)0.f;
+                    mh[(((long long)(o >> 3) * 2 + 1) * Npad + nz) * 8 + (o & 7)] = (_Float16)0.f;
+                }
+            }
+            if (mu_rows) mu_rows[(long long)n * 512 + o] = r;
+            else if (sh16 == 2)
+                mu_img[((long long)(n >> 5) * 32 + (o >> 4)) * 512 + ((n & 31) + 32 * (o & 1)) * 8 + ((o & 15) >> 1)] = r;
+            else if (sh16) {
+                _Float16* mh = reinterpret_cast<_Float16*>(mu_img);
+                _Float16 h, l;
+                sh16_split_any(r, scale, bf16, h, l);
+                vmax = fmaxf(vmax, r * scale);
+                mh[(((long long)(o >> 3) * 2 + 0) * Npad + n) * 8 + (o & 7)] = h;
+                mh[(((long long)(o >> 3) * 2 + 1) * Npad + n) * 8 + (o & 7)] = l;
+            } else mu_img[(long long)o * Npad + n] = r;
+        };
+        if constexpr (TR) {
+            float q16[16], q8[8], q4[4], q2[2];
+            const bool u5 = lane & 32, u4 = lane & 16, u3 = lane & 8, u2 = lane & 4, u1 = lane & 2;
+#pragma unroll
+            for (int v = 0; v < 16; ++v) {
+                const float lo = part[v >> 3][v & 7], hi = part[(v + 16) >> 3][v & 7];
+                q16[v] = (u5 ? hi : lo) + __shfl_xor(u5 ? lo : hi, 32, 64);
+            }
+#pragma unroll
+            for (int v = 0; v < 8; ++v) q8[v] = (u4 ? q16[v + 8] : q16[v]) + __shfl_xor(u4 ? q16[v] : q16[v + 8], 16, 64);
+#pragma unroll
+            for (int v = 0; v < 4; ++v) q4[v] = (u3 ? q8[v + 4] : q8[v]) + __shfl_xor(u3 ? q8[v] : q8[v + 4], 8, 64);
+#pragma unroll
+            for (int v = 0; v < 2; ++v) q2[v] = (u2 ? q4[v + 2] : q4[v]) + __shfl_xor(u2 ? q4[v] : q4[v + 2], 4, 64);
+            float q1 = (u1 ? q2[1] : q2[0]) + __shfl_xor(u1 ? q2[0] : q2[1], 2, 64);
+            q1 += __shfl_xor(q1, 1, 64);
+            const int v = lane >> 1;
+            if (!(lane & 1) && bb + (v & 7) < B) emit(v >> 3, v & 7, q1);
+        } else {
+#pragma unroll
             for (int i = 0; i < 4; ++i)
-                part[i][t] = w[i][0].x * c0.x + w[i][0].y * c0.y + w[i][0].z * c0.z + w[i][0].w * c0.w +
-                             w[i][1].x * c1.x + w[i][1].y * c1.y + w[i][1].z * c1.z + w[i][1].w * c1.w;
-        }
-#pragma unroll
-        for (int i = 0; i < 4; ++i)
-#pragma unroll
-            for (int t = 0; t < FCMU_BT; ++t) {
-                float v = part[i][t];
-#pragma unroll
-                for (int off = 32; off > 0; off >>= 1) v += __shfl_xor(v, off, 64);
-                part[i][t] = v;
-            }
-        if (lane == 0) {
-#pragma unroll
-            for (int i = 0; i < 4; ++i)
-#pragma unroll
-                for (int t = 0; t < FCMU_BT; ++t)
-                    if (bb + t < B) {
-                        const float v = part[i][t] + bias[j * 512 + o0 + i];
-                        const float r = v > 0.f ? v : 0.f;
-                        const int o = o0 + i, n = (bb + t) * bs + j;
-                        if (bs > 19 && j == 0) {
-                            const int nz = (bb + t) * bs + 19;
-                            if (mu_rows) mu_rows[(long long)nz * 512 + o] = 0.f;
-                            else if (sh16 == 1) {
-                                _Float16* mh = reinterpret_cast<_Float16*>(mu_img);
-                                mh[(((long long)(o >> 3) * 2 + 0) * Npad + nz) * 8 + (o & 7)] = (_Float16)0.f;
-                                mh[(((long long)(o >> 3) * 2 + 1) * Npad + nz) * 8 + (o & 7)] = (_Float16)0.f;
-                            }
-                        }
-                        if (mu_rows) mu_rows[(long long)n * 512 + o] = r;
-                        else if (sh16 == 2)
-                            mu_img[((long long)(n >> 5) * 32 + (o >> 4)) * 512 + ((n & 31) + 32 * (o & 1)) * 8 + ((o & 15) >> 1)] = r;
-                        else if (sh16) {
-                            _Float16* mh = reinterpret_cast<_Float16*>(mu_img);
-                            _Float16 h, l;
-                            sh16_split_any(r, scale, bf16, h, l);
-                            vmax = fmaxf(vmax, r * scale);
-                            mh[(((long long)(o >> 3) * 2 + 0) * Npad + n) * 8 + (o & 7)] = h;
-                            mh[(((long long)(o >> 3) * 2 + 1) * Npad + n) * 8 + (o & 7)] = l;
-                        } else mu_img[(long long)o * Npad + n] = r;
-                    }
-        }
+#pragma unroll
+                for (int t = 0; t < FCMU_BT; ++t) {
+                    float v = part[i][t];
+#pragma unroll
+                    for (int off = 32; off > 0; off >>= 1) v += __shfl_xor(v, off, 64);
+                    part[i][t] = v;
+                }
+            if (lane == 0) {
+#pragma unroll
+                for (int i = 0; i < 4; ++i)
+#pragma unroll
+                    for (int t = 0; t < FCMU_BT; ++t)
+                        if (bb + t < B) emit(i, t, part[i][t]);
+            }
+        }
+    }
+    if constexpr (TR) {
+        if (sh16 == 1 && amax && pass == 0)
+#pragma unroll
+            for (int off = 32; off > 0; off >>= 1) vmax = fmaxf(vmax, __shfl_xor(vmax, off, 64));
     }
     if (sh16 == 1 && amax && pass == 0 && lane == 0) sh16_slot_max(amax, vmax);
 }
+template <bool TR>
 __global__ __launch_bounds__(256) void fc_mu_kernel(const float* __restrict__ codes, const float* __restrict__ Wt,
                                                     const float* __restrict__ bias, float* __restrict__ mu_img, int B,
                                                     int Npad, float* __restrict__ mu_rows, int sh16, int bs, float scale,
                                                     unsigned* __restrict__ amax, int pass, int bf16) {
-    fc_mu_body(codes, Wt, bias, mu_img, B, Npad, mu_rows, sh16, bs, scale, amax, pass, bf16, blockIdx.x, blockIdx.y);
-}
+    fc_mu_body<TR>(codes, Wt, bias, mu_img, B, Npad, mu_rows, sh16, bs, scale, amax, pass, bf16, blockIdx.x, blockIdx.y);
+}
+template <bool TR>
 __global__ __launch_bounds__(256) void fc_mu_batched_kernel(const float* __restrict__ codes, const float* const* __restrict__ Wts,
                                                             const float* const* __restrict__ biases, float* __restrict__ mu_base,
                                                             long long mu_stride, int B, int Npad, int bs, float scale,
@@ -894,20 +930,20 @@
     const int a = blockIdx.z;
     const float* Wt = Wts[a];
     if (!Wt) return;
-    fc_mu_body(codes, Wt, biases[a], mu_base + a * mu_stride, B, Npad, nullptr, sh16, bs, scale, sh16 == 1 ? amax_slots + 2 * a + 1 : nullptr, pass,
+    fc_mu_body<TR>(codes, Wt, biases[a], mu_base + a * mu_stride, B, Npad, nullptr, sh16, bs, scale, sh16 == 1 ? amax_slots + 2 * a + 1 : nullptr, pass,
                bf16, blockIdx.x, blockIdx.y);
 }
 hipError_t fc_mu_batched(const float* codes, const float* const* Wts, const float* const* biases, float* mu_base,
                          long long mu_stride, int n_aces, int B, int Npad, int bs, float scale, unsigned* amax_slots, int pass,
-                         int bf16, hipStream_t s, int sh16) {
-    hipLaunchKernelGGL(fc_mu_batched_kernel, dim3(512 / 16, 19, n_aces), dim3(256), 0, s, codes, Wts, biases, mu_base, mu_stride, B,
+                         int bf16, hipStream_t s, int sh16, int transposed) {
+    hipLaunchKernelGGL(transposed ? fc_mu_batched_kernel<true> : fc_mu_batched_kernel<false>, dim3(512 / 16, 19, n_aces), dim3(256), 0, s, codes, Wts, biases, mu_base, mu_stride, B,
                        Npad, bs, scale, amax_slots, pass, bf16, sh16);
     return hipGetLastError();
 }
 
 hipError_t fc_mu(const float* codes, const float* Wt, const float* bias, float* mu_img, int B, int Npad,
-                 hipStream_t s, float* mu_rows, int sh16, int bs, float scale, unsigned* amax, int pass, int bf16) {
-    hipLaunchKernelGGL(fc_mu_kernel, dim3(512 / 16, 19), dim3(256), 0, s, codes, Wt, bias, mu_img, B, Npad, mu_rows, sh16, bs,
+                 hipStream_t s, float* mu_rows, int sh16, int bs, float scale, unsigned* amax, int pass, int bf16, int transposed) {
+    hipLaunchKernelGGL(transposed ? fc_mu_kernel<true> : fc_mu_kernel<false>, dim3(512 / 16, 19), dim3(256), 0, s, codes, Wt, bias, mu_img, B, Npad, mu_rows, sh16, bs,
                        scale, amax, pass, bf16);
     return hipGetLastError();
 }
diff --git a/ctrlhair_amd/csrc/sean_model.cpp b/ctrlhair_amd/csrc/sean_model.cpp
--- a/ctrlhair_amd/csrc/sean_model.cpp
+++ b/ctrlhair_amd/csrc/sean_model.cpp
@@ -655,6 +655,7 @@
     }
     void style_lut_groups() {
         m.lut_groups = nullptr;
+        m.lut_groups_wide = false;
         m.lut_ngroups = m.lut_group_tiles = 0;
         m.lut_group_rows = 0.0;
         if (!(m.fcmu_batched && !opt.use_sh16 && opt.lut_grouped)) return;
@@ -682,6 +683,8 @@
             m.lut_groups = B.dalloc(g.size() * sizeof(PwGroup));
             if (m.lut_groups) (void)hipMemcpy(m.lut_groups, g.data(), g.size() * sizeof(PwGroup), hipMemcpyHostToDevice);
             m.lut_ngroups = (int)g.size();
+            m.lut_groups_wide = true;
+            for (const PwGroup& e : g) m.lut_groups_wide = m.lut_groups_wide && e.HW % 256 == 0;
         }
     }
 
@@ -723,6 +726,7 @@
             m.patchbuf = B.falloc((size_t)m.patch_cap_chunks * (HID + 20) * 1024);
         }
         if (wsty4_max) m.wsty4 = B.falloc(wsty4_max);
+        m.wsty4_floats = m.wsty4 ? wsty4_max : 0;
         wino4v_buffer();
         for (int k = 0; k < 6; ++k)
             if (m.wq_level[k].qlist) {
@@ -1173,7 +1177,7 @@
         const double fl = 2.0 * 18 * a.C * STYLE * N, by = 4.0 * (18.0 * a.C * STYLE + (double)STYLE * N + 18.0 * a.C * N);
         auto tm = [&](auto launch) { prof ? timed(2, fl, by, launch) : launch(); };
         if (a.lut_rows && N <= 64 && !m.opt.batch_inv) {
-            check(fc_mu(codes, a.fcmu_w, a.fcmu_b, m.mu_img, B, npad, s, m.mu_img, 0, bs), "fc_mu");
+            check(fc_mu(codes, a.fcmu_w, a.fcmu_b, m.mu_img, B, npad, s, m.mu_img, 0, bs, 1.f, nullptr, 0, 0, m.opt.pw_wide), "fc_mu");
             tm([&] { check(lut_gemv_mfma(m.mu_img, a.lut_rows, lut_buf, N, 18 * a.C, s), "lut gemv"); });
             return q;
         }
@@ -1193,7 +1197,7 @@
                 p.in = m.mu_all + (size_t)a.index * m.mu_stride;
             } else {
                 for (int pass = 0; pass < 2; ++pass)
-                    check(fc_mu(codes, a.fcmu_w, a.fcmu_b, m.mu_img, B, npad, s, nullptr, 1, bs, SH16_ACT_SCALE, mu_slot, pass, m.opt.terms == 2), "fc_mu");
+                    check(fc_mu(codes, a.fcmu_w, a.fcmu_b, m.mu_img, B, npad, s, nullptr, 1, bs, SH16_ACT_SCALE, mu_slot, pass, m.opt.terms == 2, m.opt.pw_wide), "fc_mu");
             }
             p.act = ACT_NONE;
             p.terms = m.opt.terms;
@@ -1208,7 +1212,7 @@
             q.lut_ns = 4;
         } else {
             if (m.fcmu_batched && (N > 64 || m.opt.batch_inv)) p.in = m.mu_all + (size_t)a.index * m.mu_stride;
-            else check(fc_mu(codes, a.fcmu_w, a.fcmu_b, m.mu_img, B, npad, s), "fc_mu");
+            else check(fc_mu(codes, a.fcmu_w, a.fcmu_b, m.mu_img, B, npad, s, nullptr, 0, 19, 1.f, nullptr, 0, 0, m.opt.pw_wide), "fc_mu");
             p.npix_valid = N;
             tm([&] { check(conv_nhwc1x1(p, s), "lut gemm"); });
         }
@@ -1269,6 +1273,7 @@
         q.Cout = N;
         q.groups = static_cast<const PwGroup*>(m.lut_groups);
         q.ngroups = m.lut_ngroups;
+        q.wide = m.opt.pw_wide && m.lut_groups_wide;
         const int nrg = ((N + 31) / 32 + 3) / 4;
         timed(2, 2.0 * m.lut_group_rows * STYLE * N, 4.0 * (m.lut_group_rows * STYLE + m.lut_group_rows * N + (double)m.lut_ngroups * STYLE * N),
               [&] { check(conv_pw_grouped(q, m.lut_group_tiles * nrg, st), "style LUTs (grouped GEMM)"); });
@@ -1420,7 +1425,14 @@
         Wino4vPackParams vp;
         const bool vroute = m.wino4v_route(wino4v_pays(2 * a.C, r), q.actv, B, r, p.kout, nks, vp, true);
         timed(1, dense_flops(p), 4.0 * (npix * p.kout + npix * a.C / (io.x_up ? 4.0 : 1.0) + npix * a.C), [&] {
-            if (w.wsty) check(wino4_style_pack(q.lut, m.wsty4, B, a.C, st), "wino4_style_pack");
+            if (w.wsty) {
+                const int rows = m.opt.pw_wide ? 1 : 0;
+                if (rows && m.pad_state[m.wsty4] != 1) {
+                    check(hipMemsetAsync(m.wsty4, 0, m.wsty4_floats * sizeof(float), st), "wino4 style images: zero units");
+                    m.pad_state[m.wsty4] = 1;
+                }
+                check(wino4_style_pack(q.lut, m.wsty4, B, a.C, st, rows), "wino4_style_pack");
+            }
             if (vroute) {
                 check(wino4v_pack(vp, st), "hidden activation transform (winograd F(4x4,3x3))");
                 w.v = m.vbuf;
@@ -1699,6 +1711,7 @@
             q.Cin = w.Cin;
             q.Cout = w.Cout;
             q.HW = r * r;
+            q.wide = m.opt.pw_wide;
             timed(0, 2.0 * w.Cout * w.Cin * npix, 4.0 * (npix * w.Cin + npix * w.Cout + (double)w.Cout * w.Cin),
                   [&] { check(conv_pw(q, st), "conv 1x1"); });
             return;
@@ -1760,13 +1773,13 @@
         if (opt.use_sh16) R.check(hipMemsetAsync(amax_slots, 0, 64 * sizeof(unsigned), st), "amax slots");
         if (mode.project_all) {
             R.check(fc_mu_batched(cd, fcmu_w_ptrs, fcmu_b_ptrs, mu_all, mu_stride, n_aces, B, ((B * LABEL_NC + 31) / 32) * 32, LABEL_NC, 1.f,
-                                  nullptr, 0, 0, st, mode.grouped ? 2 : 0), "fc_mu (all ACEs)");
+                                  nullptr, 0, 0, st, mode.grouped ? 2 : 0, opt.pw_wide), "fc_mu (all ACEs)");
             if (mode.grouped) R.luts_grouped();
         } else if (fcmu_batched && opt.use_sh16) {
             const int npad_c = ((B * (LABEL_NC + 1) + 31) / 32) * 32;
             for (int pass = 0; pass < 2; ++pass)
                 R.check(fc_mu_batched(cd, fcmu_w_ptrs, fcmu_b_ptrs, mu_all, mu_stride, n_aces, B, npad_c, LABEL_NC + 1, SH16_ACT_SCALE,
-                                      amax_slots, pass, opt.terms == 2, st), "fc_mu (all ACEs)");
+                                      amax_slots, pass, opt.terms == 2, st, 1, opt.pw_wide), "fc_mu (all ACEs)");
         }
         if (mode.prepass) R.prepass();
         if (mode.ahead != ChunkMode::NONE) R.prepare_all_ahead(cd);
@@ -1920,6 +1933,7 @@
                     q.Cin = cnt[ph] * 128;
                     q.Cout = 256;
                     q.HW = (int)hw4;
+                    q.wide = opt.pw_wide;
                     ck(conv_pw(q, st), "zenc convT (phase GEMM)");
                 }
                 ck(instnorm_act_d2s(tph, z10.bias, hs, B, 256, h4, h4, 1e-5f, ACT_LRELU, st), "zenc in4 (depth-to-space)");
diff --git a/ctrlhair_amd/csrc/sean_model.h b/ctrlhair_amd/csrc/sean_model.h
--- a/ctrlhair_amd/csrc/sean_model.h
+++ b/ctrlhair_amd/csrc/sean_model.h
@@ -87,6 +87,7 @@
     int terms = 3;
     int wino = 2;
     int lut_grouped = 1;
+    int pw_wide = 1;
     int prologue = 1;
     int overlap = 0;
     int wino4_force = 0;
@@ -161,6 +162,7 @@
     std::vector<hipEvent_t> ev_join;
     std::vector<float*> actv_ahead, lut_ahead;
     void* lut_groups = nullptr;
+    bool lut_groups_wide = false;
     int lut_ngroups = 0, lut_group_tiles = 0;
     double lut_group_rows = 0.0;
     bool ahead_full = false;
@@ -187,6 +189,7 @@
     int patch_cap_chunks = 0;
     float* wsty = nullptr;
     float* wsty4 = nullptr;
+    size_t wsty4_floats = 0;
     float* vbuf = nullptr;
     size_t vbuf_bytes = 0;
     bool wino4v_route(bool pays, const float* in, int Bn, int r, int K, int nks, Wino4vPackParams& vp, bool padded = false, bool reflect = false) const;
```

Measured after the change: 587.5 images/s, median of 6. 1.03x the previous value.
